# mittagessen/conformer_ocr

Measured on AMD Instinct MI355X. Metric: text lines/sec (whole node) + CER vs reference, 96×1200 bf16 batch, higher is better.
Workload: dtype bf16; 1 GPU; cfg2: conformer D=256 L=12 heads=4 sub_ch=256, batch 32 x 96x1200 per GPU, forward + CTC greedy; batches_in_queue=1, parallelism=1 independent rank(s), weights by one RCCL broadcast, streams_per_gpu=4, hipgraph_replay=True, launched_by=in-process, gpu_max_hw_queues=4, gpu_max_hw_queues_preset_by_caller=True

## Files before the change

### conformer_ocr_amd/csrc/cocr_api.hip

```cpp
#include <hip/hip_runtime.h>

#include <algorithm>
#include <cmath>
#include <cstdarg>
#include <cstdio>
#include <cstdlib>
#include <cstring>
#include <map>
#include <string>
#include <thread>
#include <vector>

#include "../../include/cocr.h"
#include "attention.hip.h"
#include "common.hip.h"
#include "conv.hip.h"
#include "ctc.hip.h"
#include "ctc_lm.hip.h"
#include "ctc_loss.hip.h"
#include "ctc_align.hip.h"
#include "train.hip.h"
#include "train_enc.hip.h"
#include "gemm.hip.h"
#include "ffn.hip.h"
#include "rowchain_args.hip.h"
#include "pack.hip.h"
#include "frontend.hip.h"
#include "norm.hip.h"
#include "preproc.hip.h"
#include "page.hip.h"
#include "augment.hip.h"
#include "score.hip.h"

static thread_local char g_err[512] = "";
static int fail(int code, const char *fmt, ...) {
    va_list ap;
    va_start(ap, fmt);
    vsnprintf(g_err, sizeof(g_err), fmt, ap);
    va_end(ap);
    return code;
}
#define HIP_TRY(expr)                                                                                      \
    do {                                                                                                   \
        hipError_t e_ = (expr);                                                                            \
        if (e_ != hipSuccess) return fail(COCR_EHIP, "%s failed: %s (%s:%d)", #expr, hipGetErrorString(e_), __FILE__, __LINE__); \
    } while (0)

extern "C" const char *cocr_last_error(void) { return g_err; }
#ifndef COCR_SRC_HASH
#define COCR_SRC_HASH "unknown"
#endif
extern "C" const char *cocr_version(void) { return "cocr-hip 0.2 (gfx950) src=" COCR_SRC_HASH; }

struct HostTensor {
    std::vector<float> data;
    std::vector<int64_t> shape;
    bool set = false;
};

struct FfnW { size_t ln_g, ln_b, w1, b1, w2, b2; };
struct LayerW {
    FfnW ffn[2];
    size_t a_ln_g, a_ln_b, wqkv, bqkv, ub, vb, wpos, wo, bo;
    size_t c_ln_g, c_ln_b, wpw1, bpw1, dww, dwb, wpw2, bpw2;
    size_t f_ln_g, f_ln_b;
};
struct StageW { size_t dw_w, dw_b, pw_w, pw_b; };
struct BlobPlan {
    size_t w0, b0;
    std::vector<StageW> stages;
    size_t wout, bout;
    std::vector<LayerW> layers;
    size_t wdec, bdec;
    size_t total = 0;
};

template <typename E> struct DevBuf {
    E *p = nullptr;
    size_t n = 0;
    const bool pinned;
    explicit DevBuf(bool pinned_ = false) : pinned(pinned_) {}
    DevBuf(const DevBuf &) = delete;
    DevBuf &operator=(const DevBuf &) = delete;
    ~DevBuf() { release(); }
    void release() {
        if (p) (void)(pinned ? hipHostFree(p) : hipFree(p));
        p = nullptr; n = 0;
    }
    hipError_t grow(size_t need, size_t alloc = 0) {
        if (need <= n) return hipSuccess;
        release();
        alloc = std::max(need, alloc);
        void *q = nullptr;
        const hipError_t e = pinned ? hipHostMalloc(&q, alloc * sizeof(E)) : hipMalloc(&q, alloc * sizeof(E));
        if (e != hipSuccess) return e;
        p = static_cast<E *>(q); n = alloc;
        return hipSuccess;
    }
};
template <typename E> static hipError_t grow_pair(DevBuf<E> &dev, DevBuf<E> &host, size_t need, size_t alloc = 0) {
    if (need <= dev.n && need <= host.n) return hipSuccess;
    dev.release(); host.release();
    hipError_t e = dev.grow(need, alloc);
    if (e == hipSuccess && (e = host.grow(need, alloc)) != hipSuccess) dev.release();
    return e;
}

#define COCR_RING_SLOTS 16
struct UploadRing {
    DevBuf<unsigned char> dev, host{true};
    hipEvent_t ev[COCR_RING_SLOTS] = {};
    int slot = 0;
    size_t at = 0;
    ~UploadRing() {
        for (hipEvent_t e : ev)
            if (e) (void)hipEventDestroy(e);
    }
    template <typename E> hipError_t stage(size_t bytes, E *&h, E *&d) {
        const size_t need = (bytes + 15) / 16 * 16 * COCR_RING_SLOTS;
        hipError_t e = hipSuccess;
        if (need > dev.n || need > host.n) {
            if ((e = hipDeviceSynchronize()) != hipSuccess) return e;
            if ((e = grow_pair(dev, host, need, (bytes + bytes / 2 + 15) / 16 * 16 * COCR_RING_SLOTS)) != hipSuccess) return e;
        }
        slot = (slot + 1) % COCR_RING_SLOTS;
        e = ev[slot] ? hipEventSynchronize(ev[slot]) : hipEventCreateWithFlags(&ev[slot], hipEventDisableTiming);
        at = dev.n / COCR_RING_SLOTS / 16 * 16 * (size_t)slot;
        h = reinterpret_cast<E *>(host.p + at); d = reinterpret_cast<E *>(dev.p + at);
        return e;
    }
    hipError_t commit(size_t bytes, hipStream_t s) {
        const hipError_t e = hipMemcpyAsync(dev.p + at, host.p + at, bytes, hipMemcpyHostToDevice, s);
        return e != hipSuccess ? e : hipEventRecord(ev[slot], s);
    }
};

struct ProfRec { int fam; hipEvent_t a, b; };
struct TrainState;

struct cocr_model {
    cocr_hparams hp;
    int device = 0;
    int D, C, L, heads, dh, dhp, ff, ksz, ncls, H, snum;
    int rD = 0, rff = 0, rdh = 0;
    bool padded = false;
    std::vector<int> feats;
    std::map<std::string, HostTensor> host;
    std::vector<std::string> names;
    int dtype = -1;
    unsigned char *blob = nullptr;
    BlobPlan plan;
    unsigned char *packed = nullptr;
    bf16_t *fpack = nullptr;
    bool packed_stale = true;
    unsigned char *ptab = nullptr;
    size_t ptab_stride = 0;
    bool ptab_stale = true;
    cocr_model *owner = nullptr;
    unsigned long long wgen = 1, seen_wgen = 0;
    std::vector<cocr_model *> sharers;
    int capN = 0, capW = 0;
    std::vector<void *> ws_allocs;
    void *z_a = nullptr, *z_b = nullptr;
    float *x = nullptr;
    void *g_lines = nullptr;
    float *g_logits = nullptr;
    void *xn = nullptr, *hid = nullptr, *q = nullptr, *k = nullptr, *vt = nullptr, *ctx = nullptr, *glu = nullptr, *dwo = nullptr;
    size_t qkv_bytes = 0;
    int vtN = -1, vtT = -1;
    int pos_maxlen = COCR_POS_MAXLEN;
    DevBuf<unsigned char> pre_buf;
    DevBuf<unsigned char> page_buf;
    UploadRing lens_ring;
    DevBuf<int32_t> ctc_lab;
    DevBuf<float> ctc_val;
    const float *amax_logits = nullptr;
    int amax_rows = 0;
    bool amax_ok = false;
    DevBuf<float> tr_pad;
    DevBuf<unsigned char> beam_bp;
    DevBuf<unsigned char> lm_scratch;
    UploadRing target_ring;
    DevBuf<float> loss_ws;
    DevBuf<unsigned> align_ws;
    UploadRing score_ring;
    DevBuf<unsigned> score_ws;
    int score_lds_max = 64 * 1024;
    int lastN = 0, lastT = 0;
    DevBuf<float> tr_part;
    float *tr_state = nullptr;
    long tr_step = 0;
    int tr_kind = -1;
    bool use_graph = false;
    struct GraphEntry { const void *lines; float *logits; int N, W, dtype; hipStream_t s; hipGraphExec_t exec; int rows; };
    std::vector<GraphEntry> graphs, graph_seen;
    bool debug = false;
    unsigned long long *stamps = nullptr;
    bool no_pad = false;
    bool beam_ref = false;
    bool no_front96 = false;
    bool no_front32 = false;
    bool no_dw_fuse = false;
    int chain_rows = 0;
    bool no_front_chain = false;
    bool ffn_probe = false;
    int att_resident_min = 192;
    bool att_resident_long = false;
    bool att_tiled = false;
    bool no_kskip = false;
    bool chain_xcd = true;
    bool no_chain = false;
    std::map<std::string, std::pair<float *, int64_t>> taps;
    DevBuf<float> tapbuf;
    TrainState *train = nullptr;
    bool profile = false;
    std::vector<ProfRec> prof;
    std::vector<hipEvent_t> ev_pool;
};

static const char *FAMILIES[] = {"frontend_fused", "frontend_conv12", "frontend_dw", "gemm_front_pw", "gemm_front_out", "layernorm",
                                 "gemm_ffn_up", "gemm_ffn_down", "ffn_fused", "chain_ffn_qkv", "chain_front_ffn_qkv", "chain_attn_out_glu", "chain_pw2_ffn_ffn_qkv", "chain_pw2_ffn", "gemm_qkv", "attention", "gemm_attn_out", "gemm_glu",
                                 "dwconv", "gemm_pw2", "gemm_decoder", "ctc_greedy", "ctc_beam", "ctc_loss", "ffn_probe", "event_pair_overhead"};
enum { FAM_FRONT96, FAM_CONV12, FAM_FDW, FAM_FPW, FAM_FOUT, FAM_LN, FAM_FFN_UP, FAM_FFN_DOWN, FAM_FFN_FUSED, FAM_CH_FIRST, FAM_CH_FRONT, FAM_CH_A, FAM_CH_B, FAM_CH_LAST, FAM_QKV, FAM_ATTN, FAM_AOUT, FAM_GLU,
       FAM_DW, FAM_PW2, FAM_DEC, FAM_GREEDY, FAM_BEAM, FAM_LOSS, FAM_FFN_PROBE, FAM_EMPTY, FAM_COUNT };

static void drop_graphs(cocr_model *m) {
    for (auto &g : m->graphs) (void)hipGraphExecDestroy(g.exec);
    m->graphs.clear();
    m->graph_seen.clear();
}

static int out_len1(int l) { return l >= 1 ? (l - 1) / 2 + 1 : 0; }

extern "C" int32_t cocr_out_len(int32_t in_len, int32_t subsampling_factor) {
    int n = 0;
    for (int f = subsampling_factor; f > 1; f >>= 1) ++n;
    for (int i = 0; i < n; ++i) in_len = out_len1(in_len);
    return in_len;
}

static void add_name(cocr_model *m, const std::string &n) { m->names.push_back(n); m->host[n]; }

struct Switch { const char *name; bool cocr_model::*flag; int cocr_model::*count; };
static const Switch SWITCHES[] = {
    {"COCR_NO_PAD", &cocr_model::no_pad, nullptr},
    {"COCR_NO_CHAIN", &cocr_model::no_chain, nullptr},
    {"COCR_NO_FRONT_CHAIN", &cocr_model::no_front_chain, nullptr},
    {"COCR_FFN_PROBE", &cocr_model::ffn_probe, nullptr},
    {"COCR_ATT_TILED", &cocr_model::att_tiled, nullptr},
    {"COCR_ATT_RESIDENT_LONG", &cocr_model::att_resident_long, nullptr},
    {"COCR_CHAIN_XCD", &cocr_model::chain_xcd, nullptr},
    {"COCR_NO_KSKIP", &cocr_model::no_kskip, nullptr},
    {"COCR_NO_DW_FUSE", &cocr_model::no_dw_fuse, nullptr},
    {"COCR_NO_FRONT96", &cocr_model::no_front96, nullptr},
    {"COCR_NO_FRONT32", &cocr_model::no_front32, nullptr},
    {"COCR_BEAM_REF", &cocr_model::beam_ref, nullptr},
    {"COCR_ATT_RESIDENT_MIN", nullptr, &cocr_model::att_resident_min},
    {"COCR_CHAIN_ROWS", nullptr, &cocr_model::chain_rows},
    {"COCR_SCORE_LDS_MAX", nullptr, &cocr_model::score_lds_max},
};

extern "C" int cocr_create(const cocr_hparams *hp, int device, cocr_model **out) {
    if (!hp || !out) return fail(COCR_EINVAL, "null argument");
    if (hp->num_classes < 1 || hp->height < 1 || hp->encoder_dim < 1 || hp->num_encoder_layers < 1 || hp->num_attention_heads < 1)
        return fail(COCR_EINVAL, "non-positive hyper-parameter");
    if (hp->encoder_dim % hp->num_attention_heads) return fail(COCR_EINVAL, "d_model %% num_heads should be zero.");
    if ((hp->conv_kernel_size - 1) % 2 || hp->conv_kernel_size < 1) return fail(COCR_EINVAL, "kernel_size should be a odd number for 'SAME' padding");
    if (hp->conv_expansion_factor != 2) return fail(COCR_EINVAL, "Currently, Only Supports expansion_factor 2");
    int sf = hp->subsampling_factor, snum = 0;
    if (sf < 2 || (sf & (sf - 1))) return fail(COCR_EINVAL, "Sampling factor should be a power of 2.");
    for (int f = sf; f > 1; f >>= 1) ++snum;
    if (snum < 1) return fail(COCR_EINVAL, "subsampling_factor must be at least 2");
    if (hp->encoder_dim % 16) return fail(COCR_EUNSUPPORTED, "encoder_dim must be a multiple of 16 (GLU tile pairing, 16-byte rows)");
    if (hp->subsampling_conv_channels % 8) return fail(COCR_EUNSUPPORTED, "subsampling_conv_channels must be a multiple of 8");
    if (hp->encoder_dim > COCR_LN_MAX_D) return fail(COCR_EUNSUPPORTED, "encoder_dim > 1024");
    const int dh = hp->encoder_dim / hp->num_attention_heads;
    if (dh > 128) return fail(COCR_EUNSUPPORTED, "d_head > 128");
    cocr_model *m = new cocr_model();
    m->hp = *hp;
    m->device = device;
    m->D = hp->encoder_dim; m->C = hp->subsampling_conv_channels; m->L = hp->num_encoder_layers;
    m->heads = hp->num_attention_heads; m->dh = dh; m->dhp = round_up(dh, 32);
    m->ff = hp->feed_forward_expansion_factor * hp->encoder_dim; m->ksz = hp->conv_kernel_size;
    m->rD = m->D; m->rff = m->ff; m->rdh = m->dh;
    m->ncls = hp->num_classes; m->H = hp->height; m->snum = snum;
    for (const Switch &w : SWITCHES) {
        const char *e = getenv(w.name);
        if (!e) continue;
        if (w.count) m->*w.count = atoi(e);
        else m->*w.flag = m->*w.flag ? e[0] != '0' : e[0] == '1';
    }
    { const char *e = getenv("COCR_CHAIN_STAMPS"); if (e && e[0] == '1') { (void)hipHostMalloc((void **)&m->stamps, 4096 * 8); memset(m->stamps, 0, 4096 * 8); } }
    int f = hp->height;
    for (int i = 0; i < snum; ++i) { f = out_len1(f); m->feats.push_back(f); }
    char buf[256];
    add_name(m, "encoder.conv_subsample.conv.0.weight");
    add_name(m, "encoder.conv_subsample.conv.0.bias");
    for (int s = 0, idx = 2; s < snum - 1; ++s, idx += 3) {
        for (int j = 0; j < 2; ++j) {
            snprintf(buf, sizeof buf, "encoder.conv_subsample.conv.%d.weight", idx + j); add_name(m, buf);
            snprintf(buf, sizeof buf, "encoder.conv_subsample.conv.%d.bias", idx + j); add_name(m, buf);
        }
    }
    add_name(m, "encoder.conv_subsample.out.0.weight");
    add_name(m, "encoder.conv_subsample.out.0.bias");
    for (int l = 0; l < m->L; ++l) {
        auto nm = [&](const char *suffix) { snprintf(buf, sizeof buf, "encoder.layers.%d.sequential.%s", l, suffix); add_name(m, buf); };
        for (int w = 0; w < 2; ++w) {
            const char *pre = w == 0 ? "0" : "3";
            for (const char *s : {"module.sequential.0.weight", "module.sequential.0.bias", "module.sequential.1.linear.weight",
                                  "module.sequential.1.linear.bias", "module.sequential.4.linear.weight", "module.sequential.4.linear.bias"}) {
                char b2[200]; snprintf(b2, sizeof b2, "%s.%s", pre, s); nm(b2);
            }
        }
        for (const char *s : {"1.module.layer_norm.weight", "1.module.layer_norm.bias", "1.module.attention.u_bias", "1.module.attention.v_bias",
                              "1.module.attention.query_proj.linear.weight", "1.module.attention.query_proj.linear.bias",
                              "1.module.attention.key_proj.linear.weight", "1.module.attention.key_proj.linear.bias",
                              "1.module.attention.value_proj.linear.weight", "1.module.attention.value_proj.linear.bias",
                              "1.module.attention.pos_proj.linear.weight", "1.module.attention.out_proj.linear.weight",
                              "1.module.attention.out_proj.linear.bias",
                              "2.module.sequential.0.weight", "2.module.sequential.0.bias", "2.module.sequential.2.conv.weight",
                              "2.module.sequential.2.conv.bias", "2.module.sequential.4.conv.weight", "2.module.sequential.5.weight",
                              "2.module.sequential.5.bias", "2.module.sequential.5.running_mean", "2.module.sequential.5.running_var",
                              "2.module.sequential.7.conv.weight", "2.module.sequential.7.conv.bias", "4.weight", "4.bias"})
            nm(s);
    }
    add_name(m, "decoder.weight");
    add_name(m, "decoder.bias");
    *out = m;
    return COCR_OK;
}

static void free_workspace(cocr_model *m) {
    for (void *p : m->ws_allocs) (void)hipFree(p);
    m->ws_allocs.clear();
    m->capN = m->capW = 0;
    m->vtN = m->vtT = -1;
}
static void clear_taps(cocr_model *m) {
    for (auto &kv : m->taps) (void)hipFree(kv.second.first);
    m->taps.clear();
    m->tapbuf.release();
}

static void drop_weights(cocr_model *m) {
    if (!m->owner) {
        for (void *p : {(void *)m->blob, (void *)m->packed, (void *)m->ptab, (void *)m->fpack})
            if (p) (void)hipFree(p);
    } else {
        auto &sh = m->owner->sharers;
        sh.erase(std::remove(sh.begin(), sh.end(), m), sh.end());
    }
    m->owner = nullptr;
    m->blob = m->packed = m->ptab = nullptr;
    m->fpack = nullptr;
}

static void train_free(cocr_model *m);
extern "C" void cocr_destroy(cocr_model *m) {
    if (!m) return;
    (void)hipSetDevice(m->device);
    train_free(m);
    free_workspace(m);
    clear_taps(m);
    for (cocr_model *sh : m->sharers) {
        drop_graphs(sh);
        sh->owner = nullptr;
        sh->blob = sh->packed = sh->ptab = nullptr;
        sh->fpack = nullptr;
    }
    m->sharers.clear();
    drop_weights(m);
    if (m->stamps) {
        (void)hipDeviceSynchronize();
        if (m->stamps[1024]) {
            for (int w = 0; w < 8; ++w) {
                const unsigned long long *q = m->stamps + 1024 + 64 * w;
                fprintf(stderr, "chain wave %d (start +%llu):", w, q[0] - m->stamps[1024]);
                for (int i = 1; i < 64 && q[i]; ++i) fprintf(stderr, " %llu", q[i] - q[i - 1]);
                fprintf(stderr, "  total %llu\n", [&] { int i = 1; while (i < 64 && q[i]) ++i; return q[i - 1] - q[0]; }());
            }
        }
        fprintf(stderr, "frontend stamps:");
        for (int i = 129; i < 192 && m->stamps[i]; ++i) fprintf(stderr, " %llu", m->stamps[i] - m->stamps[128]);
        fprintf(stderr, "\nbeam walk cycles of the stay wave, then of extension wave 0 (pairs + reads, keys, barrier + ranks, update, tail):");
        for (int i = 240; i < 250 && m->stamps[i]; ++i) fprintf(stderr, " %llu", m->stamps[i]);
        fprintf(stderr, "\nattention stamps:");
        for (int i = 193; i < 240 && m->stamps[i]; ++i) fprintf(stderr, " %llu", m->stamps[i] - m->stamps[192]);
        fprintf(stderr, "\n");
        {
            const unsigned long long *w = m->stamps + 192 + 64;
            unsigned long long t0 = ~0ull, t1 = 0;
            int nwg = 0;
            for (int i = 0; i < 1200 && w[3 * i]; ++i) { t0 = std::min(t0, w[3 * i]); t1 = std::max(t1, w[3 * i + 1]); nwg = i + 1; }
            if (nwg) {
                fprintf(stderr, "attention workgroups %d, span %.2f us (100 MHz ticks)\n", nwg, (t1 - t0) * 0.01);
                std::map<unsigned long long, int> per_cu;
                int hist_start[32] = {0};
                double dur = 0;
                for (int i = 0; i < nwg; ++i) {
                    const unsigned long long hw = w[3 * i + 2];
                    const unsigned long long cu = ((hw >> 32) << 16) | ((hw >> 8) & 0xff) | (((hw >> 13) & 7) << 8);
                    per_cu[cu]++;
                    hist_start[std::min<unsigned long long>((w[3 * i] - t0) / 100, 31)]++;
                    dur += (w[3 * i + 1] - w[3 * i]) * 0.01;
                }
                fprintf(stderr, "  mean workgroup duration %.2f us; distinct CUs %zu; start-time histogram (1 us bins):", dur / nwg, per_cu.size());
                for (int b = 0; b < 32; ++b) fprintf(stderr, " %d", hist_start[b]);
                int cnt[8] = {0};
                for (auto &kv : per_cu) cnt[std::min(kv.second, 7)]++;
                fprintf(stderr, "\n  CUs by number of workgroups received (0..7+):");
                for (int b = 0; b < 8; ++b) fprintf(stderr, " %d", cnt[b]);
                fprintf(stderr, "\n");
            }
        }
        (void)hipHostFree(m->stamps);
    }
    if (m->tr_state) (void)hipFree(m->tr_state);
    drop_graphs(m);
    for (auto &r : m->prof) { (void)hipEventDestroy(r.a); (void)hipEventDestroy(r.b); }
    for (auto e : m->ev_pool) (void)hipEventDestroy(e);
    delete m;
}

extern "C" int cocr_set_tensor(cocr_model *m, const char *name, const void *host, int dtype, int ndim, const int64_t *shape) {
    if (!m || !name || !host) return fail(COCR_EINVAL, "null argument");
    std::string n(name);
    if (n.size() > 20 && n.compare(n.size() - 19, 19, "num_batches_tracked") == 0) return COCR_OK;
    auto it = m->host.find(n);
    if (it == m->host.end()) return fail(COCR_EINVAL, "unexpected key '%s'", name);
    if (dtype != COCR_F32) return fail(COCR_EINVAL, "tensor '%s': only float32 state is accepted", name);
    int64_t cnt = 1;
    for (int i = 0; i < ndim; ++i) cnt *= shape[i];
    it->second.shape.assign(shape, shape + ndim);
    it->second.data.assign((const float *)host, (const float *)host + cnt);
    it->second.set = true;
    return COCR_OK;
}

extern "C" int cocr_missing_tensors(cocr_model *m, char *buf, size_t buflen) {
    if (!m) return fail(COCR_EINVAL, "null argument");
    int cnt = 0;
    std::string s;
    for (auto &n : m->names)
        if (!m->host[n].set) { ++cnt; s += n; s += '\n'; }
    if (buf && buflen) { strncpy(buf, s.c_str(), buflen - 1); buf[buflen - 1] = 0; }
    return cnt;
}

static size_t esize(int dtype) { return dtype == COCR_BF16 ? 2 : 4; }

static BlobPlan make_plan(const cocr_model *m, int dtype) {
    BlobPlan p;
    size_t off = 0;
    auto take = [&](size_t bytes) { size_t o = off; off += (bytes + 255) / 256 * 256; return o; };
    const size_t es = esize(dtype);
    const int D = m->D, C = m->C, ff = m->ff;
    p.w0 = take((size_t)C * 9 * 4); p.b0 = take((size_t)C * 4);
    for (int s = 0; s < m->snum - 1; ++s) {
        StageW st;
        st.dw_w = take((size_t)C * 9 * 4); st.dw_b = take((size_t)C * 4);
        st.pw_w = take((size_t)C * C * es); st.pw_b = take((size_t)C * 4);
        p.stages.push_back(st);
    }
    const int F = m->feats.back();
    p.wout = take((size_t)D * F * C * es); p.bout = take((size_t)D * 4);
    for (int l = 0; l < m->L; ++l) {
        LayerW w;
        for (int i = 0; i < 2; ++i) {
            w.ffn[i].ln_g = take(D * 4); w.ffn[i].ln_b = take(D * 4);
            w.ffn[i].w1 = take((size_t)ff * D * es); w.ffn[i].b1 = take((size_t)ff * 4);
            w.ffn[i].w2 = take((size_t)D * ff * es); w.ffn[i].b2 = take(D * 4);
        }
        w.a_ln_g = take(D * 4); w.a_ln_b = take(D * 4);
        w.wqkv = take((size_t)3 * D * D * es); w.bqkv = take((size_t)3 * D * 4);
        w.ub = take(D * 4); w.vb = take(D * 4);
        w.wpos = take((size_t)D * D * 4);
        w.wo = take((size_t)D * D * es); w.bo = take(D * 4);
        w.c_ln_g = take(D * 4); w.c_ln_b = take(D * 4);
        w.wpw1 = take((size_t)2 * D * D * es); w.bpw1 = take((size_t)2 * D * 4);
        w.dww = take((size_t)m->ksz * D * 4); w.dwb = take(D * 4);
        w.wpw2 = take((size_t)D * D * es); w.bpw2 = take(D * 4);
        w.f_ln_g = take(D * 4); w.f_ln_b = take(D * 4);
        p.layers.push_back(w);
    }
    p.wdec = take((size_t)m->ncls * D * es); p.bdec = take((size_t)m->ncls * 4);
    p.total = off;
    return p;
}

static uint16_t f32_to_bf16(float f) {
    uint32_t u;
    memcpy(&u, &f, 4);
    if ((u & 0x7fffffffu) > 0x7f800000u) return (uint16_t)((u >> 16) | 0x40);
    u += 0x7fffu + ((u >> 16) & 1u);
    return (uint16_t)(u >> 16);
}

static void put_matrix(unsigned char *dst, int dtype, const float *src, int rows, int cols, const std::vector<int> *rowmap = nullptr,
                       const std::vector<int> *colmap = nullptr) {
    for (int r = 0; r < rows; ++r) {
        const float *s = src + (size_t)(rowmap ? (*rowmap)[r] : r) * cols;
        for (int c = 0; c < cols; ++c) {
            const float v = s[colmap ? (*colmap)[c] : c];
            if (dtype == COCR_BF16) ((uint16_t *)dst)[(size_t)r * cols + c] = f32_to_bf16(v);
            else ((float *)dst)[(size_t)r * cols + c] = v;
        }
    }
}
static void put_f32(unsigned char *dst, const float *src, size_t n) { memcpy(dst, src, n * 4); }

static int expect_shape(const cocr_model *m, const std::string &name, std::initializer_list<int64_t> shape, const HostTensor **out) {
    auto it = m->host.find(name);
    if (it == m->host.end() || !it->second.set) return fail(COCR_ESTATE, "missing tensor '%s'", name.c_str());
    if (it->second.shape != std::vector<int64_t>(shape)) {
        std::string got;
        for (auto v : it->second.shape) got += std::to_string(v) + ",";
        return fail(COCR_EINVAL, "size mismatch for %s: got (%s)", name.c_str(), got.c_str());
    }
    *out = &it->second;
    return COCR_OK;
}

static int ensure_ptab(cocr_model *m, hipStream_t s);

static void free_workspace(cocr_model *m);
static int set_engine_dims(cocr_model *m, int dtype) {
    const int wide = m->rD < 256 ? 256 : 512;
    const int slot = m->heads > 0 && wide % m->heads == 0 ? wide / m->heads : 0;
    const bool pad = dtype == COCR_BF16 && !m->no_pad && m->rD >= 128 && m->rD < 512 && m->rD != 256 && slot >= m->rdh && slot % 32 == 0 && slot <= 128 &&
                     round_up(m->rff, 256) <= (wide == 256 ? 1024 : 2048);
    const int D = pad ? wide : m->rD, ff = pad ? round_up(m->rff, 256) : m->rff, dh = pad ? slot : m->rdh, dhp = pad ? slot : round_up(m->rdh, 32);
    if (D != m->D || ff != m->ff || dh != m->dh || dhp != m->dhp) {
        HIP_TRY(hipDeviceSynchronize());
        drop_graphs(m);
        free_workspace(m);
        m->capN = m->capW = 0;
    }
    m->D = D; m->ff = ff; m->dh = dh; m->dhp = dhp; m->padded = pad;
    return COCR_OK;
}

static int alloc_blob(cocr_model *m, int dtype) {
    if (dtype != COCR_BF16 && dtype != COCR_F32) return fail(COCR_EINVAL, "compute dtype must be COCR_BF16 or COCR_F32");
    HIP_TRY(hipSetDevice(m->device));
    { const int rc = set_engine_dims(m, dtype); if (rc) return rc; }
    drop_weights(m);
    m->wgen++;
    m->ptab_stale = true;
    if (m->tr_state) { (void)hipFree(m->tr_state); m->tr_state = nullptr; m->tr_step = 0; }
    m->packed_stale = true;
    m->plan = make_plan(m, dtype);
    m->dtype = dtype;
    HIP_TRY(hipMalloc((void **)&m->blob, m->plan.total));
    HIP_TRY(hipMemset(m->blob, 0, m->plan.total));
    return COCR_OK;
}

extern "C" int cocr_finalize_empty(cocr_model *m, int compute_dtype) {
    if (!m) return fail(COCR_EINVAL, "null argument");
    int rc = alloc_blob(m, compute_dtype);
    if (rc) return rc;
    HIP_TRY(hipDeviceSynchronize());
    return COCR_OK;
}

extern "C" int cocr_share_weights(cocr_model *m, cocr_model *owner) {
    if (!m || !owner || m == owner) return fail(COCR_EINVAL, "two different models expected");
    if (owner->owner) return fail(COCR_EINVAL, "the owner itself shares another model's weights");
    if (owner->dtype < 0 || !owner->blob) return fail(COCR_ESTATE, "the owner is not finalized");
    if (m->device != owner->device || memcmp(&m->hp, &owner->hp, sizeof m->hp) != 0) return fail(COCR_EINVAL, "models of the same hyper-parameters on the same device expected");
    if (m->train || owner->train) return fail(COCR_ESTATE, "not while a training state exists");
    HIP_TRY(hipSetDevice(m->device));
    HIP_TRY(hipDeviceSynchronize());
    if (m->dtype != owner->dtype || !m->blob || m->owner) { const int rc = alloc_blob(m, owner->dtype); if (rc) return rc; }
    drop_weights(m);
    m->owner = owner;
    owner->sharers.push_back(m);
    m->seen_wgen = 0;
    m->blob = owner->blob;
    drop_graphs(m);
    return COCR_OK;
}

extern "C" int cocr_weight_blob(cocr_model *m, void **device_ptr, size_t *bytes) {
    if (!m || !device_ptr || !bytes) return fail(COCR_EINVAL, "null argument");
    if (!m->blob) return fail(COCR_ESTATE, "model not finalized");
    if (m->owner) return fail(COCR_ESTATE, "this model shares another model's weights: address the owner");
    *device_ptr = m->blob;
    *bytes = m->plan.total;
    m->packed_stale = m->ptab_stale = true;
    return COCR_OK;
}

extern "C" int cocr_blob_export(cocr_model *m, void *dst_device, size_t bytes, void *stream) {
    if (!m || !dst_device) return fail(COCR_EINVAL, "null argument");
    if (!m->blob) return fail(COCR_ESTATE, "model not finalized");
    if (m->owner) return fail(COCR_ESTATE, "this model shares another model's weights: address the owner");
    if (bytes != m->plan.total) return fail(COCR_EINVAL, "blob is %zu bytes, buffer %zu", m->plan.total, bytes);
    HIP_TRY(hipSetDevice(m->device));
    HIP_TRY(hipMemcpyAsync(dst_device, m->blob, bytes, hipMemcpyDeviceToDevice, (hipStream_t)stream));
    return COCR_OK;
}
extern "C" int cocr_blob_import(cocr_model *m, const void *src_device, size_t bytes, void *stream) {
    if (!m || !src_device) return fail(COCR_EINVAL, "null argument");
    if (!m->blob) return fail(COCR_ESTATE, "model not finalized");
    if (bytes != m->plan.total) return fail(COCR_EINVAL, "blob is %zu bytes, buffer %zu", m->plan.total, bytes);
    if (m->owner) return fail(COCR_ESTATE, "this model shares another model's weights: address the owner");
    HIP_TRY(hipSetDevice(m->device));
    HIP_TRY(hipMemcpyAsync(m->blob, src_device, bytes, hipMemcpyDeviceToDevice, (hipStream_t)stream));
    m->packed_stale = m->ptab_stale = true;
    if (m->tr_state) { (void)hipFree(m->tr_state); m->tr_state = nullptr; m->tr_step = 0; }
    return COCR_OK;
}

static void put_mapped(unsigned char *dst, int dtype, const float *src, int src_cols, const std::vector<int> &rmap, const std::vector<int> &cmap) {
    const size_t vcols = cmap.size();
    for (size_t r = 0; r < rmap.size(); ++r)
        for (size_t c = 0; c < vcols; ++c) {
            const float v = (rmap[r] >= 0 && cmap[c] >= 0) ? src[(size_t)rmap[r] * src_cols + cmap[c]] : 0.0f;
            if (dtype == COCR_BF16) ((uint16_t *)dst)[r * vcols + c] = f32_to_bf16(v);
            else ((float *)dst)[r * vcols + c] = v;
        }
}
static void put_vec(unsigned char *dst, const float *src, const std::vector<int> &map) {
    for (size_t i = 0; i < map.size(); ++i) ((float *)dst)[i] = map[i] >= 0 ? src[map[i]] : 0.0f;
}

extern "C" int cocr_finalize(cocr_model *m, int dtype) {
    if (!m) return fail(COCR_EINVAL, "null argument");
    if (dtype != COCR_BF16 && dtype != COCR_F32) return fail(COCR_EINVAL, "compute dtype must be COCR_BF16 or COCR_F32");
    HIP_TRY(hipSetDevice(m->device));
    int rc;
    if ((rc = set_engine_dims(m, dtype))) return rc;
    const int rD = m->rD, rff = m->rff, rdh = m->rdh, D = m->D, C = m->C, ff = m->ff, k = m->ksz, h = m->heads, dh = m->dh;
    std::vector<int> Mm(D), Fm(ff), Am(D), Gm((size_t)2 * D), ident_cls(m->ncls);
    for (int c = 0; c < D; ++c) Mm[c] = c < rD ? c : -1;
    for (int c = 0; c < ff; ++c) Fm[c] = c < rff ? c : -1;
    for (int c = 0; c < D; ++c) Am[c] = (c / dh < h && c % dh < rdh) ? (c / dh) * rdh + c % dh : -1;
    for (int n = 0; n < 2 * D; ++n) {
        const int tn = n >> 4, c = n & 15, j = tn >> 1, v = 16 * j + c;
        Gm[n] = v < rD ? ((tn & 1) ? rD + v : v) : -1;
    }
    for (int c = 0; c < m->ncls; ++c) ident_cls[c] = c;
    const BlobPlan plan = make_plan(m, dtype);
    std::vector<unsigned char> stage(plan.total, 0);
    unsigned char *st = stage.data();
    const HostTensor *t = nullptr;
    char buf[256];
#define GET(NAME, ...)                                          \
    if ((rc = expect_shape(m, NAME, {__VA_ARGS__}, &t))) return rc;
    GET("encoder.conv_subsample.conv.0.weight", C, 1, 3, 3); put_f32(st + plan.w0, t->data.data(), (size_t)C * 9);
    GET("encoder.conv_subsample.conv.0.bias", C); put_f32(st + plan.b0, t->data.data(), C);
    for (int s = 0, idx = 2; s < m->snum - 1; ++s, idx += 3) {
        snprintf(buf, sizeof buf, "encoder.conv_subsample.conv.%d.weight", idx); GET(buf, C, 1, 3, 3); put_f32(st + plan.stages[s].dw_w, t->data.data(), (size_t)C * 9);
        snprintf(buf, sizeof buf, "encoder.conv_subsample.conv.%d.bias", idx); GET(buf, C); put_f32(st + plan.stages[s].dw_b, t->data.data(), C);
        snprintf(buf, sizeof buf, "encoder.conv_subsample.conv.%d.weight", idx + 1); GET(buf, C, C, 1, 1); put_matrix(st + plan.stages[s].pw_w, dtype, t->data.data(), C, C);
        snprintf(buf, sizeof buf, "encoder.conv_subsample.conv.%d.bias", idx + 1); GET(buf, C); put_f32(st + plan.stages[s].pw_b, t->data.data(), C);
    }
    {
        const int F = m->feats.back();
        GET("encoder.conv_subsample.out.0.weight", rD, (int64_t)C * F);
        std::vector<int> colmap((size_t)F * C);
        for (int f = 0; f < F; ++f) for (int c = 0; c < C; ++c) colmap[(size_t)f * C + c] = c * F + f;
        put_mapped(st + plan.wout, dtype, t->data.data(), F * C, Mm, colmap);
        GET("encoder.conv_subsample.out.0.bias", rD); put_vec(st + plan.bout, t->data.data(), Mm);
    }
    for (int l = 0; l < m->L; ++l) {
        const LayerW &w = plan.layers[l];
        auto key = [&](const char *suffix) { snprintf(buf, sizeof buf, "encoder.layers.%d.sequential.%s", l, suffix); return std::string(buf); };
        for (int i = 0; i < 2; ++i) {
            const std::string pre = std::string(i == 0 ? "0" : "3") + ".module.sequential.";
            GET(key((pre + "0.weight").c_str()), rD); put_vec(st + w.ffn[i].ln_g, t->data.data(), Mm);
            GET(key((pre + "0.bias").c_str()), rD); put_vec(st + w.ffn[i].ln_b, t->data.data(), Mm);
            GET(key((pre + "1.linear.weight").c_str()), rff, rD); put_mapped(st + w.ffn[i].w1, dtype, t->data.data(), rD, Fm, Mm);
            GET(key((pre + "1.linear.bias").c_str()), rff); put_vec(st + w.ffn[i].b1, t->data.data(), Fm);
            GET(key((pre + "4.linear.weight").c_str()), rD, rff); put_mapped(st + w.ffn[i].w2, dtype, t->data.data(), rff, Mm, Fm);
            GET(key((pre + "4.linear.bias").c_str()), rD); put_vec(st + w.ffn[i].b2, t->data.data(), Mm);
        }
        GET(key("1.module.layer_norm.weight"), rD); put_vec(st + w.a_ln_g, t->data.data(), Mm);
        GET(key("1.module.layer_norm.bias"), rD); put_vec(st + w.a_ln_b, t->data.data(), Mm);
        const char *proj[3] = {"query", "key", "value"};
        for (int j = 0; j < 3; ++j) {
            snprintf(buf, sizeof buf, "encoder.layers.%d.sequential.1.module.attention.%s_proj.linear.weight", l, proj[j]);
            GET(std::string(buf), rD, rD); put_mapped(st + w.wqkv + (size_t)j * D * D * esize(dtype), dtype, t->data.data(), rD, Am, Mm);
            snprintf(buf, sizeof buf, "encoder.layers.%d.sequential.1.module.attention.%s_proj.linear.bias", l, proj[j]);
            GET(std::string(buf), rD); put_vec(st + w.bqkv + (size_t)j * D * 4, t->data.data(), Am);
        }
        GET(key("1.module.attention.u_bias"), h, rdh); put_vec(st + w.ub, t->data.data(), Am);
        GET(key("1.module.attention.v_bias"), h, rdh); put_vec(st + w.vb, t->data.data(), Am);
        GET(key("1.module.attention.pos_proj.linear.weight"), rD, rD); put_mapped(st + w.wpos, COCR_F32, t->data.data(), rD, Am, Mm);
        GET(key("1.module.attention.out_proj.linear.weight"), rD, rD); put_mapped(st + w.wo, dtype, t->data.data(), rD, Mm, Am);
        GET(key("1.module.attention.out_proj.linear.bias"), rD); put_vec(st + w.bo, t->data.data(), Mm);
        GET(key("2.module.sequential.0.weight"), rD); put_vec(st + w.c_ln_g, t->data.data(), Mm);
        GET(key("2.module.sequential.0.bias"), rD); put_vec(st + w.c_ln_b, t->data.data(), Mm);
        GET(key("2.module.sequential.2.conv.weight"), 2 * rD, rD, 1); put_mapped(st + w.wpw1, dtype, t->data.data(), rD, Gm, Mm);
        GET(key("2.module.sequential.2.conv.bias"), 2 * rD); put_vec(st + w.bpw1, t->data.data(), Gm);
        {
            const HostTensor *wd, *g, *b, *mu, *var;
            if ((rc = expect_shape(m, key("2.module.sequential.4.conv.weight"), {rD, 1, k}, &wd))) return rc;
            if ((rc = expect_shape(m, key("2.module.sequential.5.weight"), {rD}, &g))) return rc;
            if ((rc = expect_shape(m, key("2.module.sequential.5.bias"), {rD}, &b))) return rc;
            if ((rc = expect_shape(m, key("2.module.sequential.5.running_mean"), {rD}, &mu))) return rc;
            if ((rc = expect_shape(m, key("2.module.sequential.5.running_var"), {rD}, &var))) return rc;
            float *tw = (float *)(st + w.dww), *tb = (float *)(st + w.dwb);
            for (int c = 0; c < rD; ++c) {
                const float s = g->data[c] / sqrtf(var->data[c] + 1e-5f);
                for (int tau = 0; tau < k; ++tau) tw[(size_t)tau * D + c] = wd->data[(size_t)c * k + tau] * s;
                tb[c] = b->data[c] - mu->data[c] * s;
            }
        }
        GET(key("2.module.sequential.7.conv.weight"), rD, rD, 1); put_mapped(st + w.wpw2, dtype, t->data.data(), rD, Mm, Mm);
        GET(key("2.module.sequential.7.conv.bias"), rD); put_vec(st + w.bpw2, t->data.data(), Mm);
        GET(key("4.weight"), rD); put_vec(st + w.f_ln_g, t->data.data(), Mm);
        GET(key("4.bias"), rD); put_vec(st + w.f_ln_b, t->data.data(), Mm);
    }
    GET("decoder.weight", m->ncls, rD); put_mapped(st + plan.wdec, dtype, t->data.data(), rD, ident_cls, Mm);
    GET("decoder.bias", m->ncls); put_f32(st + plan.bdec, t->data.data(), m->ncls);
#undef GET
    if ((rc = alloc_blob(m, dtype))) return rc;
    HIP_TRY(hipMemcpy(m->blob, st, plan.total, hipMemcpyHostToDevice));
    if ((rc = ensure_ptab(m, nullptr))) return rc;
    HIP_TRY(hipDeviceSynchronize());
    return COCR_OK;
}

template <typename T> static int compute_pos_tables(cocr_model *m, hipStream_t s) {
    const int D = m->D, rD = m->rD, maxlen = m->pos_maxlen, R = 2 * maxlen - 1;
    std::vector<float> pe((size_t)R * D, 0.0f);
    for (int r = 0; r < R; ++r) {
        const float pos = (float)(maxlen - 1 - r);
        for (int i = 0; i < rD; i += 2) {
            const float div = expf((float)i * (float)(-(log(10000.0) / rD)));
            const float ang = pos * div;
            pe[(size_t)r * D + i] = sinf(ang);
            if (i + 1 < rD) pe[(size_t)r * D + i + 1] = cosf(ang);
        }
    }
    float *d_pe = nullptr;
    HIP_TRY(hipMalloc((void **)&d_pe, pe.size() * 4));
    HIP_TRY(hipMemcpyAsync(d_pe, pe.data(), pe.size() * 4, hipMemcpyHostToDevice, s));
    for (int l = 0; l < m->L; ++l) {
        EpiPosTable<T> epi{(T *)(m->ptab + (size_t)l * m->ptab_stride), m->dh, m->dhp, m->heads};
        HIP_TRY(launch_gemm<float>(s, d_pe, D, (const float *)(m->blob + m->plan.layers[l].wpos), D, R, D, D, epi));
    }
    HIP_TRY(hipStreamSynchronize(s));
    HIP_TRY(hipFree(d_pe));
    return COCR_OK;
}
static int ensure_ptab(cocr_model *m, hipStream_t s) {
    if (!m->ptab_stale) return COCR_OK;
    m->ptab_stride = (size_t)(2 * m->pos_maxlen - 1) * m->heads * m->dhp * esize(m->dtype);
    if (!m->ptab) {
        HIP_TRY(hipMalloc((void **)&m->ptab, m->ptab_stride * m->L));
        HIP_TRY(hipMemsetAsync(m->ptab, 0, m->ptab_stride * m->L, s));
    }
    int rc = m->dtype == COCR_BF16 ? compute_pos_tables<bf16_t>(m, s) : compute_pos_tables<float>(m, s);
    if (rc) return rc;
    m->ptab_stale = false;
    return COCR_OK;
}

static int ws_alloc(cocr_model *m, void **p, size_t bytes) {
    HIP_TRY(hipMalloc(p, bytes ? bytes : 256));
    m->ws_allocs.push_back(*p);
    return COCR_OK;
}

extern "C" int cocr_reserve(cocr_model *m, int N, int W) {
    if (!m) return fail(COCR_EINVAL, "null argument");
    if (m->dtype < 0) return fail(COCR_ESTATE, "model not finalized");
    if (N < 1 || W < 1) return fail(COCR_EINVAL, "empty batch");
    if (N <= m->capN && W <= m->capW) return COCR_OK;
    HIP_TRY(hipSetDevice(m->device));
    HIP_TRY(hipDeviceSynchronize());
    N = std::max(N, m->capN); W = std::max(W, m->capW);
    drop_graphs(m);
    free_workspace(m);
    const size_t es = esize(m->dtype);
    int T = W;
    for (int i = 0; i < m->snum; ++i) T = out_len1(T);
    const int Tz = m->snum >= 2 ? out_len1(out_len1(W)) : out_len1(W);
    const size_t M = (size_t)N * T, Tp = round_up(T, 64);
    int rc;
    const size_t zbytes = (size_t)N * Tz * m->feats[m->snum >= 2 ? 1 : 0] * m->C * es;
    if ((rc = ws_alloc(m, &m->z_a, zbytes))) return rc;
    if ((rc = ws_alloc(m, &m->z_b, zbytes))) return rc;
    if ((rc = ws_alloc(m, (void **)&m->x, (M + 128) * m->D * 4))) return rc;
    if ((rc = ws_alloc(m, &m->xn, M * m->D * es))) return rc;
    if ((rc = ws_alloc(m, &m->hid, M * m->ff * es))) return rc;
    m->qkv_bytes = (size_t)N * m->heads * Tp * m->dhp * es;
    if ((rc = ws_alloc(m, &m->q, m->qkv_bytes))) return rc;
    if ((rc = ws_alloc(m, &m->k, m->qkv_bytes))) return rc;
    if ((rc = ws_alloc(m, &m->vt, m->qkv_bytes))) return rc;
    if ((rc = ws_alloc(m, &m->ctx, M * m->D * es))) return rc;
    if ((rc = ws_alloc(m, &m->glu, M * m->D * es))) return rc;
    if ((rc = ws_alloc(m, &m->dwo, M * m->D * es))) return rc;
    if ((rc = ws_alloc(m, &m->g_lines, (size_t)N * m->H * W * 4))) return rc;
    if ((rc = ws_alloc(m, (void **)&m->g_logits, M * m->ncls * 4))) return rc;
    m->capN = N; m->capW = W;
    return COCR_OK;
}

template <typename T> __global__ void to_f32_kernel(const T *in, float *out, size_t n) {
    for (size_t i = (size_t)blockIdx.x * blockDim.x + threadIdx.x; i < n; i += (size_t)gridDim.x * blockDim.x) out[i] = to_f32(in[i]);
}
template <typename T> __global__ void tap_narrow_kernel(const T *in, float *out, size_t rows, int D, int rD, int dh, int rdh, int head_major) {
    for (size_t i = (size_t)blockIdx.x * blockDim.x + threadIdx.x; i < rows * rD; i += (size_t)gridDim.x * blockDim.x) {
        const size_t r = i / rD;
        const int c = (int)(i - r * rD);
        out[i] = to_f32(in[r * D + (head_major ? (c / rdh) * dh + c % rdh : c)]);
    }
}
template <typename T> static int tap(cocr_model *m, hipStream_t s, const std::string &name, const T *src, size_t n) {
    if (!m->debug) return COCR_OK;
    auto ends = [&](const char *suf) { const size_t l = strlen(suf); return name.size() >= l && name.compare(name.size() - l, l, suf) == 0; };
    const bool own_layout = ends(".q") || ends(".k") || ends(".v") || ends(".z2") || ends(".z3");
    const bool narrow = m->padded && !own_layout && n % (size_t)m->D == 0;
    const size_t nout = narrow ? n / m->D * m->rD : n;
    float *dst = nullptr;
    HIP_TRY(hipMalloc((void **)&dst, nout * 4));
    if (narrow) hipLaunchKernelGGL((tap_narrow_kernel<T>), dim3(256), dim3(256), 0, s, src, dst, n / m->D, m->D, m->rD, m->dh, m->rdh, ends(".ctx") ? 1 : 0);
    else hipLaunchKernelGGL((to_f32_kernel<T>), dim3(256), dim3(256), 0, s, src, dst, n);
    HIP_TRY(hipStreamSynchronize(s));
    auto it = m->taps.find(name);
    if (it != m->taps.end()) (void)hipFree(it->second.first);
    m->taps[name] = {dst, (int64_t)nout};
    return COCR_OK;
}

extern "C" int cocr_set_debug(cocr_model *m, int on) {
    if (!m) return fail(COCR_EINVAL, "null argument");
    m->debug = on != 0;
    if (!on) clear_taps(m);
    return COCR_OK;
}
extern "C" int cocr_debug_tap(cocr_model *m, const char *name, float *host_out, int64_t max_elems, int64_t *n_elems) {
    if (!m || !name) return fail(COCR_EINVAL, "null argument");
    auto it = m->taps.find(name);
    if (it == m->taps.end()) return fail(COCR_EINVAL, "no tap '%s' (debug off, or stage not run)", name);
    if (n_elems) *n_elems = it->second.second;
    if (host_out) {
        if (max_elems < it->second.second) return fail(COCR_EINVAL, "tap '%s' has %lld elements", name, (long long)it->second.second);
        HIP_TRY(hipMemcpy(host_out, it->second.first, it->second.second * 4, hipMemcpyDeviceToHost));
    }
    return COCR_OK;
}

struct ProfScope {
    cocr_model *m; hipStream_t s; ProfRec r; bool on;
    ProfScope(cocr_model *m_, hipStream_t s_, int fam) : m(m_), s(s_), on(m_->profile) {
        if (!on) return;
        r.fam = fam;
        auto get = [&]() { hipEvent_t e; if (m->ev_pool.empty()) { (void)hipEventCreate(&e); } else { e = m->ev_pool.back(); m->ev_pool.pop_back(); } return e; };
        r.a = get(); r.b = get();
        (void)hipEventRecord(r.a, s);
    }
    ~ProfScope() { if (on) { (void)hipEventRecord(r.b, s); m->prof.push_back(r); } }
};

extern "C" int cocr_profile(cocr_model *m, int on) {
    if (!m) return fail(COCR_EINVAL, "null argument");
    m->profile = on != 0;
    for (auto &r : m->prof) { m->ev_pool.push_back(r.a); m->ev_pool.push_back(r.b); }
    m->prof.clear();
    return COCR_OK;
}
extern "C" int cocr_profile_read(cocr_model *m, char *names, size_t names_len, double *ms, int64_t *launches, int max_entries) {
    if (!m) return fail(COCR_EINVAL, "null argument");
    HIP_TRY(hipSetDevice(m->device));
    HIP_TRY(hipDeviceSynchronize());
    double sum[FAM_COUNT] = {0};
    int64_t cnt[FAM_COUNT] = {0};
    for (auto &r : m->prof) {
        float t = 0.f;
        HIP_TRY(hipEventElapsedTime(&t, r.a, r.b));
        sum[r.fam] += t; cnt[r.fam]++;
    }
    std::string s;
    int n = 0;
    for (int f = 0; f < FAM_COUNT && n < max_entries; ++f) {
        if (!cnt[f]) continue;
        s += FAMILIES[f]; s += '\n';
        ms[n] = sum[f] / (double)cnt[f]; launches[n] = cnt[f];
        ++n;
    }
    if (names && names_len) { strncpy(names, s.c_str(), names_len - 1); names[names_len - 1] = 0; }
    return n;
}

#define LAUNCH_CHECK() HIP_TRY(hipGetLastError())

#define GEMM_TRY(call)                                                                                 \
    do {                                                                                               \
        hipError_t e_ = (call);                                                                        \
        if (e_ != hipSuccess) return fail(COCR_EHIP, "kernel launch failed: %s (%s:%d)", hipGetErrorString(e_), __FILE__, __LINE__); \
    } while (0)

template <typename T, int DHP>
static hipError_t launch_attention(hipStream_t s, int N, const T *q, const T *k, const T *v, const T *ptab, const float *ub,
                                   const float *vb, T *ctx, int Tn, int Tp, int heads, int dh, float scale, int pos_center, unsigned long long *stamps = nullptr,
                                   bool tiled_only = false, int resident_min = 192, bool resident_long = false) {
    if constexpr (sizeof(T) == 2 && DHP == 64) {
        const int ntiles = ceil_div(Tn, 16), nqb = ceil_div(ntiles, AF_QT);
        if (dh == DHP && (Tn <= AF_TK || resident_long) && !tiled_only && !stamps && nqb * N * heads >= resident_min) {
            const int Tk0 = round_up(Tn, 64), npass = ceil_div(Tk0, AF_TK), Tk = round_up(ceil_div(Tk0, npass), 64);
            const int ntw = ceil_div(ntiles, nqb);
            const size_t lds = (size_t)(2 * Tk + 16 * ntw + Tk) * 128 + AF_WAVES * AF_SROWS * AF_SK * sizeof(float);
            auto kern = npass > 1 ? relpos_attention_full_kernel<true> : relpos_attention_full_kernel<false>;
            hipError_t e = raise_lds_limit((const void *)kern, lds);
            if (e != hipSuccess) return e;
            hipLaunchKernelGGL(kern, dim3(nqb, N * heads), dim3(64 * AF_WAVES), lds, s, (const bf16_t *)q, (const bf16_t *)k, (const bf16_t *)v,
                               (const bf16_t *)ptab, ub, vb, (bf16_t *)ctx, Tn, Tp, heads, scale * 1.44269504088896340736f, pos_center, ntw, Tk);
            return hipGetLastError();
        }
    }
    const size_t lds = attention_lds_bytes<T, DHP>();
    auto kern = relpos_attention_kernel<T, DHP>;
    hipError_t e = raise_lds_limit((const void *)kern, lds);
    if (e != hipSuccess) return e;
    hipLaunchKernelGGL(kern, dim3(ceil_div(Tn, 64), N * heads), dim3(256), lds, s, q, k, v, ptab, ub, vb, ctx, Tn, Tp, heads, dh,
                       scale * 1.44269504088896340736f, pos_center, stamps);
    return hipGetLastError();
}

static int ensure_ctc_scratch(cocr_model *m, size_t rows);

enum FrontForm {
    FRONT_96,
    FRONT_CONV0,
    FRONT_PW32,
    FRONT_MFMA,
    FRONT_VALU,
};
enum OutForm {
    OUT_IN_CHAIN,
    OUT_SPLITK,
    OUT_GEMM,
};
struct Form {
    FrontForm front;
    OutForm out;
    bool rowln;
    bool chain;
    bool ffn_fused;
    bool dw_fused;
    bool taps;
    bool argmax;
    int chain_rows;
};

static int hw_queue_count() {
    static const int n = [] {
        const char *e = getenv("GPU_MAX_HW_QUEUES");
        char *end = nullptr;
        long v = e ? strtol(e, &end, 10) : 4;
        if (e && (end == e || *end)) v = 4;
        return (int)std::min(32L, std::max(1L, v));
    }();
    return n;
}

static int chain_rows_for(const cocr_model *m, int M) {
    const bool d256 = m->D == 256;
    auto form = [&](int hint) { return 16 * (d256 ? rowchain_pick_mt<256>(M, hint) : rowchain_pick_mt<512>(M, hint)); };
    if (m->chain_rows > 0) return form(m->chain_rows);
    const cocr_model *root = m->owner ? m->owner : m;
    const int S = 1 + (int)root->sharers.size();
    if (S < 2) return form(0);
    const int Q = std::max(1, hw_queue_count() - 1), turns = ceil_div(S, Q);
    static const int forms256[] = {96, 64, 48}, forms512[] = {64};
    const int *forms = d256 ? forms256 : forms512, nforms = d256 ? 3 : 1;
    int rows = 32;
    for (int i = 0; i < nforms; ++i) {
        if (M < 50 * forms[i]) continue;
        rows = forms[i];
        if ((long)ceil_div(M, rows) * S >= 256L * turns) break;
    }
    return rows;
}

#ifndef COCR_FO_SPLITS
#define COCR_FO_SPLITS 2
#endif
static Form forward_form(const cocr_model *m, int N, int W) {
    const bool bf16 = m->dtype == COCR_BF16, f2only = m->snum == 1;
    const int es = bf16 ? 2 : 4, D = m->D, C = m->C, H = m->H;
    const int T1 = out_len1(W), T2 = f2only ? T1 : out_len1(T1), F2 = m->feats[f2only ? 0 : 1];
    const int Kf = m->feats.back() * C, M = N * cocr_out_len(W, m->hp.subsampling_factor);
    const size_t lds32 = (size_t)(4 * 16 + 3) * ((H + 11) & ~3) * 4 + (size_t)16 * F2 * 80;
    Form f{};
    f.taps = m->debug;
    f.rowln = bf16 ? gemm_rowln_supported<bf16_t>(D) : gemm_rowln_supported<float>(D);
    f.chain = bf16 && rowchain_supported(D, m->ff, m->dh) && !m->no_chain;
    if (bf16 && m->snum == 2 && frontend96_supported(C, m->feats[0], m->feats[1], H) && !m->no_front96) f.front = FRONT_96;
    else if (f2only) f.front = FRONT_CONV0;
    else if (bf16 && C == 32 && F2 <= 32 && lds32 <= 160 * 1024 && !f.taps && !m->no_front32) f.front = FRONT_PW32;
    else f.front = bf16 && C % 64 == 0 ? FRONT_MFMA : FRONT_VALU;
    if (f.chain && Kf % 256 == 0 && !m->no_front_chain) f.out = OUT_IN_CHAIN;
    else if (f.rowln && Kf % (COCR_FO_SPLITS * (128 / es)) == 0 && D <= 256 && (size_t)COCR_FO_SPLITS * M * D * 4 <= (size_t)N * T2 * F2 * C * es)
        f.out = OUT_SPLITK;
    else f.out = OUT_GEMM;
    f.ffn_fused = bf16 && f.rowln && ffn_fused_supported<int>(D, m->ff);
    f.dw_fused = m->ksz == 31 && (!m->no_dw_fuse || f.taps);
    f.argmax = m->ncls <= 128 && D % (128 / es) == 0;
    f.chain_rows = f.chain ? chain_rows_for(m, M) : 0;
    return f;
}

template <typename T> struct Fwd {
    cocr_model *m;
    const Form &f;
    hipStream_t s;
    const BlobPlan &P;
    const int N, W, D, T1, T2, F1, F2, Tn, M, Tp;
    const float ffr, scale;
    T *const za, *const zb;
    float *const x;
    T *const xn, *const hid, *const q, *const k, *const v, *const ctx, *const glu, *const dwo;
    Fwd(cocr_model *m_, const Form &f_, int N_, int W_, hipStream_t s_)
        : m(m_), f(f_), s(s_), P(m_->plan), N(N_), W(W_), D(m_->D), T1(out_len1(W_)), T2(m_->snum == 1 ? T1 : out_len1(T1)), F1(m_->feats[0]),
          F2(m_->feats[m_->snum == 1 ? 0 : 1]), Tn(cocr_out_len(W_, m_->hp.subsampling_factor)), M(N_ * Tn), Tp(round_up(Tn, 64)),
          ffr(m_->hp.half_step_residual ? 0.5f : 1.0f), scale(1.0f / sqrtf((float)m_->rdh)), za((T *)m_->z_a), zb((T *)m_->z_b), x(m_->x),
          xn((T *)m_->xn), hid((T *)m_->hid), q((T *)m_->q), k((T *)m_->k), v((T *)m_->vt), ctx((T *)m_->ctx), glu((T *)m_->glu), dwo((T *)m_->dwo) {}
    const float *F32(size_t off) const { return (const float *)(m->blob + off); }
    const T *WT(size_t off) const { return (const T *)(m->blob + off); }
    template <typename S> int tap(int l, const char *what, const S *src, size_t n) const {
        if (!f.taps) return COCR_OK;
        char nm[64];
        if (l < 0) snprintf(nm, sizeof nm, "%s", what);
        else snprintf(nm, sizeof nm, "l%d.%s", l, what);
        return ::tap<S>(m, s, nm, src, n);
    }
    int tap_x(int l, const char *what, const float *src) const { return tap<float>(l, what, src, (size_t)M * D); }
    int tap_qkv(int l) const {
        const size_t n = m->qkv_bytes / sizeof(T);
        int rc;
        if ((rc = tap<T>(l, "q", q, n)) || (rc = tap<T>(l, "k", k, n)) || (rc = tap<T>(l, "v", v, n))) return rc;
        return COCR_OK;
    }
};

template <typename T, typename TIn> static int frontend(const Fwd<T> &c, const TIn *lines) {
    cocr_model *m = c.m;
    const BlobPlan &P = c.P;
    const hipStream_t s = c.s;
    const int N = c.N, H = m->H, W = c.W, C = m->C, T1 = c.T1, F1 = c.F1, T2 = c.T2, F2 = c.F2;
    const FrontForm form = c.f.front;
    T *za = c.za, *zb = c.zb;
    int rc;
    if (form == FRONT_CONV0) {
        ProfScope ps(m, s, FAM_CONV12);
        const size_t npos = (size_t)N * T1 * F1;
        hipLaunchKernelGGL((frontend_conv0_kernel<T, TIn>), dim3((unsigned)((npos * (size_t)(C / 2) + 255) / 256)), dim3(256), 0, s, lines, H, W, T1, F1, C, npos,
                           c.F32(P.w0), c.F32(P.b0), zb);
        LAUNCH_CHECK();
        return COCR_OK;
    }
    if (form == FRONT_96) {
        ProfScope ps(m, s, FAM_FRONT96);
        const size_t n0 = (size_t)(C / 16) * 64 * 4;
        GEMM_TRY(launch_frontend96<TIn>(s, lines, N, H, W, T1, F1, T2, m->fpack, c.F32(P.b0), m->fpack + n0, c.F32(P.stages[0].dw_b),
                                        (const bf16_t *)(m->packed + P.stages[0].pw_w), c.F32(P.stages[0].pw_b), (bf16_t *)zb, m->stamps ? m->stamps + 128 : nullptr));
    } else if (form == FRONT_PW32) {
        ProfScope ps(m, s, FAM_CONV12);
        const size_t lds = (size_t)(4 * 16 + 3) * ((H + 11) & ~3) * 4 + (size_t)16 * F2 * 80;
        auto kern = frontend_conv12pw32_kernel<TIn>;
        GEMM_TRY(raise_lds_limit((const void *)kern, lds));
        hipLaunchKernelGGL(kern, dim3(ceil_div(T2, 16), N), dim3(256), lds, s, lines, H, W, T1, F1, T2, F2, c.F32(P.w0), c.F32(P.b0),
                           c.F32(P.stages[0].dw_w), c.F32(P.stages[0].dw_b), (const bf16_t *)c.WT(P.stages[0].pw_w), c.F32(P.stages[0].pw_b), (bf16_t *)zb);
        LAUNCH_CHECK();
    } else {
        {
            ProfScope ps(m, s, FAM_CONV12);
            if (form == FRONT_MFMA) {
                GEMM_TRY(launch_conv12_mfma<TIn>(s, lines, N, H, W, T1, F1, T2, F2, C, c.F32(P.w0), c.F32(P.b0), c.F32(P.stages[0].dw_w), c.F32(P.stages[0].dw_b),
                                                 (bf16_t *)za));
            } else {
                const int TB = std::max(1, 512 / C);
                const size_t lds = (size_t)(4 * TB + 3) * ((H + 11) & ~3) * 4;
                hipLaunchKernelGGL((frontend_conv12_kernel<T, TIn>), dim3(ceil_div(T2, TB), N), dim3(256), lds, s, lines, H, W, T1, F1, T2, F2, C,
                                   c.F32(P.w0), c.F32(P.b0), c.F32(P.stages[0].dw_w), c.F32(P.stages[0].dw_b), za, TB);
                LAUNCH_CHECK();
            }
        }
        if ((rc = c.tap(-1, "front.z2", za, (size_t)N * T2 * F2 * C))) return rc;
        ProfScope ps(m, s, FAM_FPW);
        EpiBiasAct<T, ACT_RELU> epi{zb, C, c.F32(P.stages[0].pw_b), C};
        GEMM_TRY(launch_gemm<T>(s, za, C, c.WT(P.stages[0].pw_w), C, N * T2 * F2, C, C, epi));
    }
    if ((rc = c.tap(-1, "front.z3", zb, (size_t)N * T2 * F2 * C))) return rc;
    int Tc = T2, Fc = F2;
    for (int st = 1; st < m->snum - 1; ++st) {
        const int To = out_len1(Tc), Fo = m->feats[st + 1];
        {
            ProfScope ps(m, s, FAM_FDW);
            hipLaunchKernelGGL((dw3x3s2_kernel<T>), dim3(1024), dim3(256), 0, s, zb, N, Tc, Fc, To, Fo, C, c.F32(P.stages[st].dw_w),
                               c.F32(P.stages[st].dw_b), za);
            LAUNCH_CHECK();
        }
        {
            ProfScope ps(m, s, FAM_FPW);
            EpiBiasAct<T, ACT_RELU> epi{zb, C, c.F32(P.stages[st].pw_b), C};
            GEMM_TRY(launch_gemm<T>(s, za, C, c.WT(P.stages[st].pw_w), C, N * To * Fo, C, C, epi));
        }
        Tc = To; Fc = Fo;
    }
    return COCR_OK;
}

template <typename T> static int layernorm(const Fwd<T> &c, size_t g1, size_t b1, bool write_f32, long g2, long b2) {
    ProfScope ps(c.m, c.s, FAM_LN);
    launch_layernorm<T>(c.s, c.x, c.M, c.D, c.F32(g1), c.F32(b1), write_f32 ? c.x : nullptr, g2 >= 0 ? c.F32((size_t)g2) : nullptr,
                        b2 >= 0 ? c.F32((size_t)b2) : nullptr, c.xn, c.m->rD);
    LAUNCH_CHECK();
    return COCR_OK;
}

template <typename T> static int gemm_to_stream(const Fwd<T> &c, int fam, const T *A, int K, size_t w, size_t bias, float alpha, bool resid,
                                                size_t g1, size_t b1, long g2, long b2) {
    const int M = c.M, D = c.D;
    {
        ProfScope ps(c.m, c.s, fam);
        if (c.f.rowln) {
            EpiResidualLN<T, 1> e{c.x, D, c.F32(bias), alpha, D, resid ? 1 : 0, c.F32(g1), c.F32(b1), g2 >= 0 ? c.F32((size_t)g2) : nullptr,
                                  b2 >= 0 ? c.F32((size_t)b2) : nullptr, c.xn};
            e.Dn = c.m->rD;
            GEMM_TRY(launch_gemm_rowln<T>(c.s, A, K, c.WT(w), K, M, D, K, e));
            return COCR_OK;
        }
        if (resid) { EpiResidual e{c.x, D, c.F32(bias), alpha, D}; GEMM_TRY(launch_gemm<T>(c.s, A, K, c.WT(w), K, M, D, K, e)); }
        else { EpiStoreF32 e{c.x, D, c.F32(bias), D}; GEMM_TRY(launch_gemm<T>(c.s, A, K, c.WT(w), K, M, D, K, e)); }
    }
    return layernorm(c, g1, b1, g2 >= 0, g2, b2);
}

template <typename T> static int front_out(const Fwd<T> &c) {
    cocr_model *m = c.m;
    const BlobPlan &P = c.P;
    const FfnW &f0 = P.layers[0].ffn[0];
    const int Kf = m->feats.back() * m->C, M = c.M, D = c.D;
    if (c.f.out == OUT_IN_CHAIN) return COCR_OK;
    if (c.f.out == OUT_SPLITK) {
        float *partial = reinterpret_cast<float *>(c.za);
        { ProfScope ps(m, c.s, FAM_FOUT); GEMM_TRY(launch_gemm_splitk<T>(c.s, c.zb, Kf, c.WT(P.wout), Kf, M, D, Kf, COCR_FO_SPLITS, partial)); }
        ProfScope ps(m, c.s, FAM_LN);
        hipLaunchKernelGGL((splitk_reduce_ln_kernel<T>), dim3(ceil_div(M, 16)), dim3(256), 0, c.s, partial, COCR_FO_SPLITS, (size_t)M * D, c.F32(P.bout), M, D,
                           m->rD, c.F32(f0.ln_g), c.F32(f0.ln_b), c.x, c.xn);
        LAUNCH_CHECK();
    } else {
        const int rc = gemm_to_stream(c, FAM_FOUT, c.zb, Kf, P.wout, P.bout, 1.0f, false, f0.ln_g, f0.ln_b, -1, -1);
        if (rc) return rc;
    }
    return c.tap_x(-1, "front.y", c.x);
}

template <typename T> static int ffn_up(const Fwd<T> &c, const FfnW &fw) {
    ProfScope ps(c.m, c.s, FAM_FFN_UP);
    EpiBiasAct<T, ACT_SILU> e{c.hid, c.m->ff, c.F32(fw.b1), c.m->ff};
    GEMM_TRY(launch_gemm<T>(c.s, c.xn, c.D, c.WT(fw.w1), c.D, c.M, c.m->ff, c.D, e));
    return COCR_OK;
}
template <typename T> static int ffn(const Fwd<T> &c, const FfnW &fw, size_t g1, size_t b1, long g2, long b2) {
    if constexpr (sizeof(T) == 2) {
        if (c.f.ffn_fused) {
            ProfScope ps(c.m, c.s, FAM_FFN_FUSED);
            EpiResidualLN<T, 1> e{c.x, c.D, c.F32(fw.b2), c.ffr, c.D, 1, c.F32(g1), c.F32(b1), g2 >= 0 ? c.F32((size_t)g2) : nullptr,
                                  b2 >= 0 ? c.F32((size_t)b2) : nullptr, c.xn};
            GEMM_TRY(launch_ffn_fused(c.s, (const bf16_t *)c.xn, (const bf16_t *)c.WT(fw.w1), c.F32(fw.b1), (const bf16_t *)c.WT(fw.w2), c.M, c.D, c.m->ff, e));
            return COCR_OK;
        }
    }
    const int rc = ffn_up(c, fw);
    return rc ? rc : gemm_to_stream(c, FAM_FFN_DOWN, c.hid, c.m->ff, fw.w2, fw.b2, c.ffr, true, g1, b1, g2, b2);
}

template <typename T, int DHP> static hipError_t attention_dhp(const Fwd<T> &c, int l, unsigned long long *stamps) {
    const cocr_model *m = c.m;
    const LayerW &w = c.P.layers[l];
    return launch_attention<T, DHP>(c.s, c.N, c.q, c.k, c.v, (const T *)(m->ptab + (size_t)l * m->ptab_stride), c.F32(w.ub), c.F32(w.vb), c.ctx, c.Tn,
                                    c.Tp, m->heads, m->dh, c.scale, m->pos_maxlen - 1, stamps, m->att_tiled, m->att_resident_min, m->att_resident_long);
}
template <typename T> static int attention(const Fwd<T> &c, int l, unsigned long long *stamps) {
    ProfScope ps(c.m, c.s, FAM_ATTN);
    const int dhp = c.m->dhp;
    GEMM_TRY((dhp == 32   ? attention_dhp<T, 32>(c, l, stamps)
              : dhp == 64 ? attention_dhp<T, 64>(c, l, stamps)
              : dhp == 96 ? attention_dhp<T, 96>(c, l, stamps)
                          : attention_dhp<T, 128>(c, l, stamps)));
    return COCR_OK;
}

template <typename T> static int dwconv(const Fwd<T> &c, const LayerW &w) {
    ProfScope ps(c.m, c.s, FAM_DW);
    launch_dwconv<T>(c.s, c.glu, c.N, c.Tn, c.D, c.m->ksz, c.F32(w.dww), c.F32(w.dwb), c.dwo);
    LAUNCH_CHECK();
    return COCR_OK;
}

template <typename T> static int encoder_products(const Fwd<T> &c) {
    cocr_model *m = c.m;
    const hipStream_t s = c.s;
    const int M = c.M, D = c.D;
    const size_t MD = (size_t)M * D;
    int rc;
    for (int l = 0; l < m->L; ++l) {
        const LayerW &w = c.P.layers[l];
        const bool last = l + 1 == m->L;
        const long g_next = last ? -1 : (long)c.P.layers[l + 1].ffn[0].ln_g, b_next = last ? -1 : (long)c.P.layers[l + 1].ffn[0].ln_b;
        if ((rc = ffn(c, w.ffn[0], w.a_ln_g, w.a_ln_b, -1, -1)) || (rc = c.tap_x(l, "ffn1", c.x))) return rc;
        { ProfScope ps(m, s, FAM_QKV); EpiQKV<T> e{c.q, c.k, c.v, c.F32(w.bqkv), D, m->dh, m->dhp, m->heads, c.Tn, c.Tp, 3 * D}; GEMM_TRY(launch_gemm<T>(s, c.xn, D, c.WT(w.wqkv), D, M, 3 * D, D, e)); }
        if ((rc = attention(c, l, nullptr)) || (rc = c.tap_qkv(l)) || (rc = c.tap(l, "ctx", c.ctx, MD))) return rc;
        if ((rc = gemm_to_stream(c, FAM_AOUT, c.ctx, D, w.wo, w.bo, 1.0f, true, w.c_ln_g, w.c_ln_b, -1, -1)) || (rc = c.tap_x(l, "mhsa", c.x))) return rc;
        { ProfScope ps(m, s, FAM_GLU); EpiGLU<T> e{c.glu, D, c.F32(w.bpw1), 2 * D}; GEMM_TRY(launch_gemm<T>(s, c.xn, D, c.WT(w.wpw1), D, M, 2 * D, D, e)); }
        if ((rc = dwconv(c, w)) || (rc = c.tap(l, "glu", c.glu, MD)) || (rc = c.tap(l, "dw", c.dwo, MD))) return rc;
        if ((rc = gemm_to_stream(c, FAM_PW2, c.dwo, D, w.wpw2, w.bpw2, 1.0f, true, w.ffn[1].ln_g, w.ffn[1].ln_b, -1, -1)) || (rc = c.tap_x(l, "conv", c.x))) return rc;
        if (!c.f.taps) {
            if ((rc = ffn(c, w.ffn[1], w.f_ln_g, w.f_ln_b, g_next, b_next))) return rc;
            continue;
        }
        if ((rc = ffn_up(c, w.ffn[1]))) return rc;
        { ProfScope ps(m, s, FAM_FFN_DOWN); EpiResidual e{c.x, D, c.F32(w.ffn[1].b2), c.ffr, D}; GEMM_TRY(launch_gemm<T>(s, c.hid, m->ff, c.WT(w.ffn[1].w2), m->ff, M, D, m->ff, e)); }
        if ((rc = c.tap_x(l, "ffn2", c.x)) || (rc = layernorm(c, w.f_ln_g, w.f_ln_b, true, g_next, b_next)) || (rc = c.tap_x(l, "out", c.x))) return rc;
    }
    return COCR_OK;
}

template <typename T> static int encoder_chains(const Fwd<T> &c) {
    cocr_model *m = c.m;
    const BlobPlan &P = c.P;
    const int D = c.D, M = c.M;
    const size_t MD = (size_t)M * D;
    const bool taps = c.f.taps;
    int rc;
    float *tp[4] = {nullptr, nullptr, nullptr, nullptr};
    bf16_t *tap_dw = nullptr;
    if (taps) {
        HIP_TRY(m->tapbuf.grow(MD * 4 + MD / 2));
        for (int i = 0; i < 4; ++i) tp[i] = m->tapbuf.p + (size_t)i * MD;
        tap_dw = reinterpret_cast<bf16_t *>(m->tapbuf.p + 4 * MD);
    }
    auto CW = [&](size_t off) { return (const bf16_t *)(m->packed + off); };
    auto launch = [&](const ChainArgs &a, int fam) -> int {
        ProfScope ps(m, c.s, fam);
        GEMM_TRY(D == 256 ? launch_rowchain_256(c.s, a, taps, c.f.chain_rows) : launch_rowchain_512(c.s, a, taps, c.f.chain_rows));
        return COCR_OK;
    };
    auto base = [&](const T *A0, int nstages) {
        ChainArgs a{}; a.x = c.x; a.x_in_blocked = 1; a.x_out_blocked = 1; a.xn = (bf16_t *)c.xn; a.M = M; a.dh = m->dh; a.dhp = m->dhp; a.heads = m->heads; a.T_ = c.Tn; a.Tp = c.Tp; a.inv_d = 1.0f / (float)m->rD; a.xcd_order = m->chain_xcd ? 1 : 0;
        a.kd = (m->padded && !m->no_kskip) ? ceil_div(m->rD, 32) : 8; a.kl = (m->padded && !m->no_kskip) ? ((m->rff - 1) % 256) / 32 + 1 : 8;
        a.A0 = (const bf16_t *)A0; a.nstages = nstages; return a; };
    auto st_rowln = [&](size_t wgt, size_t bias, float alpha, size_t g1, size_t b1) {
        ChainStage st{}; st.kind = ST_ROWLN; st.W = CW(wgt); st.bias = c.F32(bias); st.N = D; st.alpha = alpha;
        st.g1 = c.F32(g1); st.b1 = c.F32(b1); return st; };
    auto st_ffn = [&](const FfnW &fw, size_t g1, size_t b1, long g2, long b2) {
        ChainStage st{}; st.kind = ST_FFN; st.W = CW(fw.w1); st.W2 = CW(fw.w2); st.bias = c.F32(fw.b1); st.bias2 = c.F32(fw.b2);
        st.N = m->ff; st.alpha = c.ffr; st.g1 = c.F32(g1); st.b1 = c.F32(b1);
        st.g2 = g2 >= 0 ? c.F32((size_t)g2) : nullptr; st.b2 = b2 >= 0 ? c.F32((size_t)b2) : nullptr; return st; };
    auto st_qkv = [&](const LayerW &lw) {
        ChainStage st{}; st.kind = ST_QKV; st.W = CW(lw.wqkv); st.bias = c.F32(lw.bqkv); st.N = 3 * D;
        st.q = (bf16_t *)c.q; st.k = (bf16_t *)c.k; st.v = (bf16_t *)c.v; return st; };
    const LayerW &w0 = P.layers[0];
    if (c.f.out == OUT_IN_CHAIN) {
        ChainArgs a = base(c.zb, 3); a.x_in_blocked = 0;
        ChainStage f{}; f.kind = ST_FRONT; f.W = CW(P.wout); f.bias = c.F32(P.bout); f.N = D; f.K = m->feats.back() * m->C; f.alpha = 1.0f;
        f.g1 = c.F32(w0.ffn[0].ln_g); f.b1 = c.F32(w0.ffn[0].ln_b);
        a.st[0] = f;
        a.st[1] = st_ffn(w0.ffn[0], w0.a_ln_g, w0.a_ln_b, -1, -1); a.st[1].store_x = 1;
        a.st[2] = st_qkv(w0);
        a.st[0].tap_pre = tp[1]; a.st[1].tap_pre = tp[0];
        if ((rc = launch(a, FAM_CH_FRONT)) || (rc = c.tap_x(-1, "front.y", tp[1])) || (rc = c.tap_x(0, "ffn1", tp[0])) || (rc = c.tap_qkv(0))) return rc;
    } else {
        ChainArgs a = base(c.xn, 2); a.x_in_blocked = 0;
        a.st[0] = st_ffn(w0.ffn[0], w0.a_ln_g, w0.a_ln_b, -1, -1); a.st[0].store_x = 1;
        a.st[1] = st_qkv(w0);
        a.st[0].tap_pre = tp[0];
        if ((rc = launch(a, FAM_CH_FIRST)) || (rc = c.tap_x(0, "ffn1", tp[0])) || (rc = c.tap_qkv(0))) return rc;
    }
    if (m->ffn_probe) {
        ChainArgs a = base(c.zb, 1);
        a.st[0] = st_ffn(w0.ffn[0], w0.a_ln_g, w0.a_ln_b, -1, -1);
        if ((rc = launch(a, FAM_FFN_PROBE))) return rc;
    }
    for (int l = 0; l < m->L; ++l) {
        const LayerW &w = P.layers[l];
        const bool last = l + 1 == m->L;
        if ((rc = attention(c, l, (m->stamps && l == 5) ? m->stamps + 192 : nullptr))) return rc;
        {
            ChainArgs a = base(c.ctx, 2);
            a.st[0] = st_rowln(w.wo, w.bo, 1.0f, w.c_ln_g, w.c_ln_b); a.st[0].store_x = 1;
            ChainStage g{}; g.kind = ST_GLU; g.W = CW(w.wpw1); g.bias = c.F32(w.bpw1); g.N = 2 * D; g.out = (bf16_t *)c.glu;
            a.st[1] = g;
            a.st[0].tap_pre = tp[0];
            if ((rc = c.tap(l, "ctx", c.ctx, MD)) || (rc = launch(a, FAM_CH_A)) || (rc = c.tap_x(l, "mhsa", tp[0])) || (rc = c.tap(l, "glu", c.glu, MD))) return rc;
        }
        if (!c.f.dw_fused && (rc = dwconv(c, w))) return rc;
        ChainArgs a = base(c.dwo, 2);
        if (c.f.dw_fused) { a.dw_in = (const bf16_t *)c.glu; a.dw_w = c.F32(w.dww); a.dw_b = c.F32(w.dwb); a.tap_dw = tap_dw; }
        a.st[0] = st_rowln(w.wpw2, w.bpw2, 1.0f, w.ffn[1].ln_g, w.ffn[1].ln_b);
        a.st[0].tap_pre = tp[0];
        if (!last) {
            const LayerW &nx = P.layers[l + 1];
            a.st[1] = st_ffn(w.ffn[1], w.f_ln_g, w.f_ln_b, (long)nx.ffn[0].ln_g, (long)nx.ffn[0].ln_b);
            a.st[2] = st_ffn(nx.ffn[0], nx.a_ln_g, nx.a_ln_b, -1, -1); a.st[2].store_x = 1;
            a.st[3] = st_qkv(nx);
            a.nstages = 4;
            a.st[1].tap_pre = tp[1]; a.st[1].tap_post = tp[2]; a.st[2].tap_pre = tp[3];
            a.stamps = (m->stamps && l == 5) ? m->stamps + 1024 : nullptr;
            if ((rc = launch(a, FAM_CH_B))) return rc;
        } else {
            a.st[1] = st_ffn(w.ffn[1], w.f_ln_g, w.f_ln_b, -1, -1); a.st[1].store_x = 1; a.st[1].store_xn = 1;
            a.st[1].tap_pre = tp[1];
            if ((rc = launch(a, FAM_CH_LAST))) return rc;
        }
        if ((rc = c.tap(l, "dw", c.f.dw_fused ? (const T *)tap_dw : (const T *)c.dwo, MD)) || (rc = c.tap_x(l, "conv", tp[0])) || (rc = c.tap_x(l, "ffn2", tp[1])))
            return rc;
        if (!last && ((rc = c.tap_x(l, "out", tp[2])) || (rc = c.tap_x(l + 1, "ffn1", tp[3])) || (rc = c.tap_qkv(l + 1)))) return rc;
        if (last && (rc = c.tap(l, "out", c.xn, MD))) return rc;
    }
    return COCR_OK;
}

template <typename T> static int decoder(const Fwd<T> &c, float *logits) {
    cocr_model *m = c.m;
    const int M = c.M, D = c.D;
    ProfScope ps(m, c.s, FAM_DEC);
    if (c.f.argmax) {
        const int rc = ensure_ctc_scratch(m, (size_t)M);
        if (rc) return rc;
        EpiLogitsArgmax e{logits, m->ncls, c.F32(c.P.bdec), m->ncls, m->ctc_lab.p, m->ctc_val.p};
        GemmArgs<T> a{c.xn, D, c.WT(c.P.wdec), D, M, m->ncls, D, 0};
        GEMM_TRY((launch_ring_cfg<T, 64, 128, 3, EpiLogitsArgmax>(c.s, a, e)));
        m->amax_ok = true; m->amax_rows = M;
        return COCR_OK;
    }
    EpiStoreF32 e{logits, m->ncls, c.F32(c.P.bdec), m->ncls};
    GEMM_TRY(launch_gemm<T>(c.s, c.xn, D, c.WT(c.P.wdec), D, M, m->ncls, D, e));
    m->amax_ok = false;
    return COCR_OK;
}

template <typename T, typename TIn>
static int forward_impl(cocr_model *m, const Form &f, const TIn *lines, int N, int W, float *logits, hipStream_t s) {
    const Fwd<T> c(m, f, N, W, s);
    { ProfScope ps(m, s, FAM_EMPTY); }
    int rc;
    if ((rc = frontend<T, TIn>(c, lines)) || (rc = front_out(c))) return rc;
    if (m->vtN != N || m->vtT != c.Tn) {
        for (T *p : {c.q, c.k, c.v}) HIP_TRY(hipMemsetAsync(p, 0, m->qkv_bytes, s));
        m->vtN = N; m->vtT = c.Tn;
    }
    if constexpr (sizeof(T) == 2) rc = f.chain ? encoder_chains(c) : encoder_products(c);
    else rc = encoder_products(c);
    return rc ? rc : decoder(c, logits);
}

static int ensure_packed(cocr_model *m, const Form &f, hipStream_t s) {
    if ((!f.chain && f.front != FRONT_96) || !m->packed_stale) return COCR_OK;
    if (!m->packed) HIP_TRY(hipMalloc((void **)&m->packed, m->plan.total));
    const int D = m->D, ff = m->ff, C = m->C;
    auto pack = [&](size_t off, int N, int K, float scale = 1.0f) {
        hipLaunchKernelGGL(pack_frag_kernel, dim3(std::min(1024, ceil_div(N * K / 8, 256))), dim3(256), 0, s, (const bf16_t *)(m->blob + off),
                           (bf16_t *)(m->packed + off), N, K, scale);
    };
    const float ffr = m->hp.half_step_residual ? 0.5f : 1.0f;
    if (f.chain)
        for (const LayerW &w : m->plan.layers) {
            for (int i = 0; i < 2; ++i) { pack(w.ffn[i].w1, ff, D); pack(w.ffn[i].w2, D, ff, ffr); }
            pack(w.wqkv, 3 * D, D); pack(w.wo, D, D); pack(w.wpw1, 2 * D, D); pack(w.wpw2, D, D);
        }
    if (f.out == OUT_IN_CHAIN) pack(m->plan.wout, D, m->feats.back() * C);
    if (f.front == FRONT_96) {
        pack(m->plan.stages[0].pw_w, C, C);
        const size_t n0 = (size_t)(C / 16) * 64 * 4, n2 = (size_t)(C / 16) * 5 * 64 * 8;
        if (!m->fpack) HIP_TRY(hipMalloc((void **)&m->fpack, (n0 + n2) * sizeof(bf16_t)));
        hipLaunchKernelGGL(frontend_pack_kernel, dim3(ceil_div((int)n2, 256)), dim3(256), 0, s, (const float *)(m->blob + m->plan.w0),
                           (const float *)(m->blob + m->plan.stages[0].dw_w), m->fpack, m->fpack + n0, C);
    }
    LAUNCH_CHECK();
    m->packed_stale = false;
    drop_graphs(m);
    return COCR_OK;
}

static int forward_entry(cocr_model *m, const void *lines, int line_dtype, int N, int H, int W, const int32_t *in_lens,
                         float *logits, int32_t *out_lens, void *stream);
extern "C" int cocr_forward(cocr_model *m, const void *lines, int line_dtype, int N, int H, int W, const int32_t *in_lens,
                            float *logits, int32_t *out_lens, void *stream) {
    if (m) m->amax_logits = nullptr;
    const int rc = forward_entry(m, lines, line_dtype, N, H, W, in_lens, logits, out_lens, stream);
    if (rc == COCR_OK && m->amax_ok) m->amax_logits = logits;
    return rc;
}
extern "C" int cocr_forget_argmax(cocr_model *m) {
    if (!m) return fail(COCR_EINVAL, "null argument");
    m->amax_logits = nullptr;
    return COCR_OK;
}
static int forward_entry(cocr_model *m, const void *lines, int line_dtype, int N, int H, int W, const int32_t *in_lens,
                         float *logits, int32_t *out_lens, void *stream) {
    if (!m || !lines || !logits) return fail(COCR_EINVAL, "null argument");
    if (m->dtype < 0 || !m->blob) return fail(COCR_ESTATE, "model not finalized");
    if (H != m->H) return fail(COCR_EINVAL, "line height %d does not match the model's height %d", H, m->H);
    if (N < 1 || W < 1) return fail(COCR_EINVAL, "empty batch");
    HIP_TRY(hipSetDevice(m->device));
    {
        const int Tp64 = round_up(cocr_out_len(W, m->hp.subsampling_factor), 64);
        if (Tp64 > 65536) return fail(COCR_EUNSUPPORTED, "more than 65536 output frames");
        cocr_model *root = m->owner ? m->owner : m;
        if (Tp64 + 64 > root->pos_maxlen) {
            HIP_TRY(hipDeviceSynchronize());
            drop_graphs(m);
            if (root->ptab) { (void)hipFree(root->ptab); root->ptab = nullptr; }
            root->pos_maxlen = round_up(Tp64 + 64, 1024);
            root->ptab_stale = true;
            root->wgen++;
        }
    }
    int rc;
    if (m->owner && (m->owner->dtype != m->dtype || m->owner->plan.total != m->plan.total)) {
        cocr_model *o = m->owner;
        if (o->dtype < 0 || !o->blob) return fail(COCR_ESTATE, "the model whose weights this one shares is not finalized");
        HIP_TRY(hipDeviceSynchronize());
        if ((rc = set_engine_dims(m, o->dtype))) return rc;
        drop_graphs(m);
        free_workspace(m);
        m->plan = make_plan(m, o->dtype);
        m->dtype = o->dtype;
        m->blob = o->blob;
        m->amax_logits = nullptr;
        m->seen_wgen = 0;
    }
    rc = cocr_reserve(m, N, W);
    if (rc) return rc;
    if (in_lens && out_lens)
        for (int i = 0; i < N; ++i) out_lens[i] = cocr_out_len(in_lens[i], m->hp.subsampling_factor);
    hipStream_t s = (hipStream_t)stream;
    const Form form = forward_form(m, N, W);
    if (m->owner) {
        cocr_model *o = m->owner;
        if (o->packed_stale || o->ptab_stale) {
            HIP_TRY(hipDeviceSynchronize());
            if ((rc = ensure_packed(o, form, s)) || (rc = ensure_ptab(o, s))) return rc;
            HIP_TRY(hipDeviceSynchronize());
            o->wgen++;
        }
        if (m->seen_wgen != o->wgen) {
            m->blob = o->blob; m->packed = o->packed; m->fpack = o->fpack; m->ptab = o->ptab; m->ptab_stride = o->ptab_stride; m->pos_maxlen = o->pos_maxlen;
            m->packed_stale = m->ptab_stale = false;
            m->seen_wgen = o->wgen;
            drop_graphs(m);
        }
    } else {
        const bool rebuilt = m->packed_stale || m->ptab_stale;
        if (rebuilt && m->wgen > 1) HIP_TRY(hipDeviceSynchronize());
        if ((rc = ensure_packed(m, form, s)) || (rc = ensure_ptab(m, s))) return rc;
        if (rebuilt) { m->wgen++; HIP_TRY(hipStreamSynchronize(s)); }
        if (m->seen_wgen != m->wgen) {
            if (m->seen_wgen) drop_graphs(m);
            m->seen_wgen = m->wgen;
        }
    }
    m->lastN = N;
    m->lastT = cocr_out_len(W, m->hp.subsampling_factor);
    auto run_on = [&](const void *in, float *out) -> int {
        if (m->dtype == COCR_BF16) {
            if (line_dtype == COCR_F32) return forward_impl<bf16_t, float>(m, form, (const float *)in, N, W, out, s);
            if (line_dtype == COCR_U8) return forward_impl<bf16_t, uint8_t>(m, form, (const uint8_t *)in, N, W, out, s);
        } else {
            if (line_dtype == COCR_F32) return forward_impl<float, float>(m, form, (const float *)in, N, W, out, s);
            if (line_dtype == COCR_U8) return forward_impl<float, uint8_t>(m, form, (const uint8_t *)in, N, W, out, s);
        }
        return fail(COCR_EINVAL, "line dtype must be COCR_F32 or COCR_U8");
    };
    auto run = [&]() -> int { return run_on(lines, logits); };
    if (line_dtype != COCR_F32 && line_dtype != COCR_U8) return fail(COCR_EINVAL, "line dtype must be COCR_F32 or COCR_U8");
    if (!m->use_graph || m->debug || m->profile || s == nullptr) return run();
    const int Tn = cocr_out_len(W, m->hp.subsampling_factor);
    const bool shape_ready = m->vtN == N && m->vtT == Tn;
    auto same = [&](const cocr_model::GraphEntry &g) { return g.lines == lines && g.logits == logits && g.N == N && g.W == W && g.dtype == line_dtype; };
    auto same_shape = [&](const cocr_model::GraphEntry &g) { return g.lines == nullptr && g.N == N && g.W == W && g.dtype == line_dtype; };
    auto capture = [&](const void *in, float *out, hipGraphExec_t *exec) -> int {
        hipGraph_t graph = nullptr;
        HIP_TRY(hipStreamBeginCapture(s, hipStreamCaptureModeThreadLocal));
        int r = run_on(in, out);
        hipError_t ce = hipStreamEndCapture(s, &graph);
        if (r) { if (graph) (void)hipGraphDestroy(graph); return r; }
        if (ce != hipSuccess) return fail(COCR_EHIP, "hipStreamEndCapture failed: %s", hipGetErrorString(ce));
        HIP_TRY(hipGraphInstantiate(exec, graph, nullptr, nullptr, 0));
        (void)hipGraphDestroy(graph);
        if (m->graphs.size() >= 16) { (void)hipGraphExecDestroy(m->graphs.front().exec); m->graphs.erase(m->graphs.begin()); }
        return COCR_OK;
    };
    const size_t in_bytes = (size_t)N * H * W * (line_dtype == COCR_F32 ? 4 : 1), out_bytes = (size_t)N * Tn * m->ncls * 4;
    auto staged_launch = [&](hipGraphExec_t exec) -> int {
        HIP_TRY(hipMemcpyAsync(m->g_lines, lines, in_bytes, hipMemcpyDefault, s));
        HIP_TRY(hipGraphLaunch(exec, s));
        HIP_TRY(hipMemcpyAsync(logits, m->g_logits, out_bytes, hipMemcpyDeviceToDevice, s));
        return COCR_OK;
    };
    for (auto &g : m->graphs)
        if (g.N == N && g.W == W && g.rows != form.chain_rows) {
            drop_graphs(m);
            break;
        }
    for (auto &g : m->graphs)
        if (same(g)) { HIP_TRY(hipGraphLaunch(g.exec, s)); return COCR_OK; }
    bool seen = false, seen_shape = false;
    for (auto &g : m->graph_seen) { seen = seen || same(g); seen_shape = seen_shape || same_shape(g); }
    if (seen && shape_ready) {
        hipGraphExec_t exec = nullptr;
        if ((rc = capture(lines, logits, &exec))) return rc;
        m->graphs.push_back({lines, logits, N, W, line_dtype, s, exec, form.chain_rows});
        HIP_TRY(hipGraphLaunch(exec, s));
        return COCR_OK;
    }
    if (m->graph_seen.size() >= 32) m->graph_seen.erase(m->graph_seen.begin());
    m->graph_seen.push_back({lines, logits, N, W, line_dtype, s, nullptr, 0});
    for (auto &g : m->graphs)
        if (same_shape(g)) return staged_launch(g.exec);
    if (!seen_shape || !shape_ready) {
        m->graph_seen.push_back({nullptr, nullptr, N, W, line_dtype, s, nullptr, 0});
        return run();
    }
    hipGraphExec_t exec = nullptr;
    if ((rc = capture(m->g_lines, m->g_logits, &exec))) return rc;
    m->graphs.push_back({nullptr, nullptr, N, W, line_dtype, s, exec, form.chain_rows});
    return staged_launch(exec);
}

extern "C" int cocr_collate_lines(const void *const *lines, const int32_t *widths, int N, int H, int elem_size, void *dst, int W, int threads) {
    if (N < 0 || H <= 0 || W <= 0 || (elem_size != 1 && elem_size != 4)) return fail(COCR_EINVAL, "collate: bad shape or element size");
    if (N == 0) return COCR_OK;
    if (!lines || !widths || !dst) return fail(COCR_EINVAL, "collate: null argument");
    for (int i = 0; i < N; ++i)
        if (!lines[i] || widths[i] < 0 || widths[i] > W) return fail(COCR_EINVAL, "collate: line %d is %d wide, the batch %d", i, widths[i], W);
    const long rows = (long)N * H;
    auto span = [=](long r0, long r1) {
        for (long r = r0; r < r1; ++r) {
            const int i = (int)(r / H), y = (int)(r % H);
            const size_t wb = (size_t)widths[i] * elem_size, Wb = (size_t)W * elem_size;
            char *d = (char *)dst + (size_t)r * Wb;
            memcpy(d, (const char *)lines[i] + (size_t)y * wb, wb);
            memset(d + wb, 0, Wb - wb);
        }
    };
    const int nt = (int)std::max(1L, std::min<long>(std::min(threads, 64), rows / 64));
    if (nt <= 1) { span(0, rows); return COCR_OK; }
    std::vector<std::thread> pool;
    pool.reserve(nt - 1);
    for (int t = 1; t < nt; ++t) pool.emplace_back(span, rows * t / nt, rows * (t + 1) / nt);
    span(0, rows / nt);
    for (auto &t : pool) t.join();
    return COCR_OK;
}

static int upload_lens(cocr_model *m, const int32_t *lens, int N, hipStream_t s, const int32_t *&d_lens) {
    int32_t *h, *d;
    HIP_TRY(m->lens_ring.stage((size_t)N * 4, h, d));
    memcpy(h, lens, (size_t)N * 4);
    HIP_TRY(m->lens_ring.commit((size_t)N * 4, s));
    d_lens = d;
    return COCR_OK;
}

static int ensure_ctc_scratch(cocr_model *m, size_t rows) {
    if (rows <= m->ctc_lab.n && rows <= m->ctc_val.n) return COCR_OK;
    HIP_TRY(hipDeviceSynchronize());
    drop_graphs(m);
    m->amax_logits = nullptr;
    HIP_TRY(m->ctc_lab.grow(rows));
    HIP_TRY(m->ctc_val.grow(rows));
    return COCR_OK;
}

extern "C" int cocr_ctc_greedy(cocr_model *m, const float *logits, int N, int T, int ncls, const int32_t *out_lens, int32_t *labels,
                               int32_t *starts, int32_t *ends, float *conf, int32_t *counts, int max_per_line, void *stream) {
    if (!m || !logits || !out_lens || !labels || !starts || !ends || !conf || !counts) return fail(COCR_EINVAL, "null argument");
    if (N < 1 || T < 1 || ncls < 1 || max_per_line < 1) return fail(COCR_EINVAL, "empty problem");
    if (T > 8000) return fail(COCR_EUNSUPPORTED, "more than 8000 frames per line");
    HIP_TRY(hipSetDevice(m->device));
    hipStream_t s = (hipStream_t)stream;
    const int32_t *d_lens;
    int rc = upload_lens(m, out_lens, N, s, d_lens);
    if (rc) return rc;
    const bool have_argmax = logits == m->amax_logits && N * T == m->amax_rows && ncls == m->ncls;
    if (!have_argmax && (rc = ensure_ctc_scratch(m, (size_t)N * T))) return rc;
    ProfScope ps(m, s, FAM_GREEDY);
    if (!have_argmax) {
        m->amax_logits = nullptr;
        hipLaunchKernelGGL(ctc_argmax_kernel, dim3(ceil_div(N * T, 4)), dim3(256), 0, s, logits, T, ncls, N * T, d_lens, m->ctc_lab.p, m->ctc_val.p);
        LAUNCH_CHECK();
    }
    hipLaunchKernelGGL(ctc_collapse_kernel, dim3(N), dim3(64), (size_t)T * 8, s, T, d_lens, m->ctc_lab.p, m->ctc_val.p, labels, starts, ends, conf, counts,
                       max_per_line);
    LAUNCH_CHECK();
    return COCR_OK;
}

extern "C" int cocr_ctc_beam(cocr_model *m, const float *logits, int N, int T, int ncls, const int32_t *out_lens, int32_t *labels,
                             int32_t *starts, int32_t *ends, float *conf, int32_t *counts, int max_per_line, int beam, void *stream) {
    if (!m || !logits || !out_lens || !labels || !starts || !ends || !conf || !counts) return fail(COCR_EINVAL, "null argument");
    if (N < 1 || T < 1 || ncls < 2 || max_per_line < 1) return fail(COCR_EINVAL, "empty problem");
    if (beam < 1 || beam > COCR_BEAM_MAX) return fail(COCR_EINVAL, "beam must be in 1..%d", COCR_BEAM_MAX);
    if (ncls > 65535) return fail(COCR_EUNSUPPORTED, "more than 65535 classes");
    HIP_TRY(hipSetDevice(m->device));
    hipStream_t s = (hipStream_t)stream;
    const int32_t *d_lens;
    int rc = upload_lens(m, out_lens, N, s, d_lens);
    if (rc) return rc;
    const bool fast = ncls <= 256 && !m->beam_ref;
    const int K = std::min(beam + 1, ncls - 1);
    const size_t need = (size_t)N * T * ((size_t)COCR_BEAM_MAX * 4 + (fast ? (size_t)COCR_BEAM_REC : 4));
    HIP_TRY(m->beam_bp.grow(need));
    int32_t *bp = reinterpret_cast<int32_t *>(m->beam_bp.p);
    ProfScope ps(m, s, FAM_BEAM);
    if (fast) {
// ... 576 lines not shown
```

### conformer_ocr_amd/csrc/rowchain.hip.h

```cpp
#pragma once
#include <type_traits>

#include "gemm.hip.h"
#include "rowchain_args.hip.h"

#ifndef COCR_STAMP_WG
#define COCR_STAMP_WG 7
#endif
#ifndef COCR_RC_EXP
#define COCR_RC_EXP 0
#endif

__device__ __forceinline__ void swap32(float &a, float &b) { asm("s_nop 1\n\tv_permlane32_swap_b32 %0, %1" : "+v"(a), "+v"(b)); }
__device__ __forceinline__ void swap16(float &a, float &b) { asm("s_nop 1\n\tv_permlane16_swap_b32 %0, %1" : "+v"(a), "+v"(b)); }
__device__ __forceinline__ float butterfly4(float a, float b, float c, float d) {
    swap32(a, b);
    swap32(c, d);
    float ab = a + b, cd = c + d;
    swap16(ab, cd);
    return ab + cd;
}

__device__ __forceinline__ int xcd_remap_rows(int bid, int nwg) {
    const int q = nwg >> 3, r = nwg & 7, xcd = bid & 7;
    return (xcd < r ? xcd * (q + 1) : r * (q + 1) + (xcd - r) * q) + (bid >> 3);
}

#ifndef COCR_RC_PAIR
#define COCR_RC_PAIR 0
#endif
template <int D, int MT> constexpr bool rowchain_pair_form() { return COCR_RC_PAIR && D == 256 && MT == 3; }

template <int D, int MT> constexpr size_t rowchain_slack_bytes() { return rowchain_pair_form<D, MT>() ? 2048 : 4096; }
template <int D, int MT> constexpr size_t rowchain_lds_bytes() {
    return (size_t)(D / 64) * 16 * MT * 128 + 2 * 4 * (size_t)(16 * MT) * 128 + rowchain_slack_bytes<D, MT>() + 16 * (size_t)D + 12 * (size_t)(16 * MT) + 64;
}
template <int D, int MT> constexpr int rowchain_dw_pass() { return rowchain_pair_form<D, MT>() ? 128 : 256; }
template <int D, int MT, int DWK> constexpr int rowchain_taps_place() {
    if (DWK == 0 || (DWK + 1) % 8 != 0) return 0;
    constexpr size_t cw = rowchain_dw_pass<D, MT>(), rpi = 64 / (cw / 8);
    constexpr size_t hsb = 2 * 4 * (size_t)(16 * MT) * 128 + rowchain_slack_bytes<D, MT>(), win = ((16 * MT + DWK - 1 + rpi - 1) / rpi) * 1024, taps = (size_t)(DWK + 1) * cw * 4;
    if (win + taps <= hsb) return 1;
    if (rowchain_pair_form<D, MT>()) return 0;
    if (rowchain_lds_bytes<D, MT>() + taps <= 160 * 1024) return 2;
    return 0;
}

template <int D, int MT, int DWK, int K0, int K1, int K2, int K3, bool TAPS, int KD = 8, int KL = 8>
__global__ __launch_bounds__(512, (rowchain_pair_form<D, MT>() ? 4 : 2)) void rowchain_kernel(ChainArgs p) {
    typedef bf16_t T;
    static_assert(D == 256 || D == 512, "encoder_dim of the row-chain kernels");
    static_assert(MT >= 2 && MT <= 6, "16-row tiles per workgroup");
    static_assert(KD >= 1 && KD <= 8 && KL >= 1 && KL <= 8 && (D == 256 || (KD == 8 && KL == 8)), "skipped k-steps: the 256-wide engine only");
    typedef std::integral_constant<int, 8> KK8;
    typedef std::integral_constant<int, KD> KKD;
    typedef std::integral_constant<int, KL> KKL;
    typedef KKD KKQ;
    typedef KKD KKG;
    typedef KKD KKP1;
    typedef std::integral_constant<int, (K1 == ST_GLU) ? 8 : KD> KKR;
    constexpr int BMC = 16 * MT;
    constexpr int KS = D / 256;
    constexpr int NS = D / 256;
    constexpr int NJ = 2 * NS;
    constexpr int PANEL = BMC * 128;
    constexpr int IMGX = (D / 64) * PANEL;
    constexpr int IMGH = 4 * PANEL;
    constexpr int OS = 256 * 2 + 16;
    constexpr int OSD = D * 2 + 16;
    constexpr int SLICE = 16 * 512;
    constexpr int PROW = 80;
    constexpr int HSB = 2 * IMGH + (int)rowchain_slack_bytes<D, MT>();
    extern __shared__ __attribute__((aligned(16))) unsigned char smem[];
    unsigned char *xa = smem;
    unsigned char *hs = smem + IMGX;
    float *lnp = reinterpret_cast<float *>(smem + IMGX + HSB);
    long long *rowoff = reinterpret_cast<long long *>(smem + IMGX + HSB + 16 * D);
    int *tpos = reinterpret_cast<int *>(smem + IMGX + HSB + 16 * D + 8 * BMC);

    const int tid = threadIdx.x, lane = tid & 63;
    const int wave = __builtin_amdgcn_readfirstlane(tid >> 6);
    const int r16 = lane & 15, g = lane >> 4, swz = r16 & 7;
    const int rblk = p.xcd_order ? xcd_remap_rows(blockIdx.x, gridDim.x) : (int)blockIdx.x;
    const int M = p.M, m0 = rblk * BMC, mend = min(M, m0 + BMC);
    const int lrow = lane >> 3, cpos = lane & 7;
#ifdef COCR_CHAIN_STAMPS_BUILD
    int sk = 0;
#define RSTAMP() { if (p.stamps && rblk == COCR_STAMP_WG && lane == 0) p.stamps[wave * 64 + sk] = __builtin_readcyclecounter(); ++sk; }
#else
#define RSTAMP()
#endif
    RSTAMP()
    auto lds_fence_barrier = [&]() {
        asm volatile("s_waitcnt lgkmcnt(0)" ::: "memory");
        if constexpr (!(COCR_RC_EXP & 512)) __builtin_amdgcn_s_barrier();
    };

    constexpr int DWPAD = DWK ? (DWK - 1) / 2 : 0, DWROWS = BMC + 2 * DWPAD;
    constexpr int CW = rowchain_dw_pass<D, MT>();
    constexpr int WS = CW * 2;
    constexpr int LPR = CW / 8, RPI = 64 / LPR;
    constexpr int WINB = ((DWROWS + RPI - 1) / RPI) * 1024;
    static_assert(DWK == 0 || (size_t)WINB <= (size_t)HSB, "depthwise window (CW channels at a time) must fit the hidden-image area");
    static_assert((size_t)BMC * OSD <= (size_t)HSB && 2 * (size_t)BMC * OS <= (size_t)HSB, "output tiles alias the hidden-image area");
    auto dw_window = [&](int h) {
        for (int q2 = wave; q2 < WINB / 1024; q2 += 8) {
            const int j = RPI * q2 + lane / LPR, mrow = min(max(m0 - DWPAD + j, 0), M - 1);
            __builtin_amdgcn_global_load_lds((gbl_ptr_t)(p.dw_in + (size_t)mrow * D + h * CW + (lane % LPR) * 8), (lds_ptr_t)(hs + q2 * 1024), 16, 0, 0);
        }
    };
    constexpr bool FRONT0 = K0 == ST_FRONT;
    static_assert(!FRONT0 || DWK == 0, "the output linear starts a launch");
    static_assert(K1 != ST_FRONT && K2 != ST_FRONT && K3 != ST_FRONT, "FRONT is a first stage");
    auto front_dma = [&](int ks) {
        unsigned char *buf = hs + (ks & 1) * IMGH;
        const int Kf = p.st[0].K;
#pragma unroll
        for (int u = 0; u < MT; ++u) {
            const int id = wave + 8 * u, pnl = id / (BMC / 8), rg = id - pnl * (BMC / 8), row = rg * 8 + lrow;
            const T *src = p.A0 + (size_t)min(m0 + row, M - 1) * Kf + ks * 256 + pnl * 64 + ((cpos ^ (row & 7)) * 8);
            __builtin_amdgcn_global_load_lds((gbl_ptr_t)src, (lds_ptr_t)(buf + pnl * PANEL + rg * 1024), 16, 0, 0);
        }
    };
    static_assert(4 * (BMC / 8) == 8 * MT, "operand slice: MT wave-instructions per wave");
    if constexpr (FRONT0) {
        front_dma(0);
    } else if constexpr (DWK == 0) {
        for (int id = wave; id < (D / 64) * (BMC / 8); id += 8) {
            const int pnl = id / (BMC / 8), rg = id - pnl * (BMC / 8), row = rg * 8 + lrow;
            const T *src = p.A0 + (size_t)min(m0 + row, M - 1) * D + pnl * 64 + ((cpos ^ (row & 7)) * 8);
            __builtin_amdgcn_global_load_lds((gbl_ptr_t)src, (lds_ptr_t)(xa + pnl * PANEL + rg * 1024), 16, 0, 0);
        }
    } else {
        dw_window(0);
    }
    typedef float dw_f32x2 __attribute__((ext_vector_type(2)));
    dw_f32x2 dw_wt[DWK ? DWK : 1], dw_bias = {0.f, 0.f};
    constexpr int TAPLACE = rowchain_taps_place<D, MT, DWK>();
    unsigned char *tapa = TAPLACE == 1 ? hs + WINB : smem + rowchain_lds_bytes<D, MT>();
    constexpr int TPI = 256 / CW;
    auto dw_taps = [&](int h) {
        if constexpr (DWK != 0 && TAPLACE != 0) {
#pragma unroll
            for (int r2 = wave; r2 < (DWK + 1) / TPI; r2 += 8) {
                const int r = r2 * TPI + lane / (64 / TPI);
                const float *src = (r < DWK ? p.dw_w + (size_t)r * D : p.dw_b) + h * CW + (lane % (64 / TPI)) * 4;
                __builtin_amdgcn_global_load_lds((gbl_ptr_t)src, (lds_ptr_t)(tapa + r2 * 1024), 16, 0, 0);
            }
        } else if constexpr (DWK != 0) {
            const int c = h * CW + 2 * (tid % (CW / 2));
#pragma unroll
            for (int tau = 0; tau < DWK; ++tau) dw_wt[tau] = *reinterpret_cast<const dw_f32x2 *>(p.dw_w + (size_t)tau * D + c);
            dw_bias = *reinterpret_cast<const dw_f32x2 *>(p.dw_b + c);
        }
    };
    auto dw_taps_read = [&]() {
        if constexpr (DWK != 0 && TAPLACE != 0) {
            const unsigned char *tb = tapa + (tid % (CW / 2)) * 8;
#pragma unroll
            for (int tau = 0; tau < DWK; ++tau) dw_wt[tau] = *reinterpret_cast<const dw_f32x2 *>(tb + tau * (CW * 4));
            dw_bias = *reinterpret_cast<const dw_f32x2 *>(tb + DWK * (CW * 4));
        }
    };
    RSTAMP()
    dw_taps(0);
    RSTAMP()
    constexpr int RING = rowchain_pair_form<D, MT>() ? 8 : 16;
    bf16x8 ring[RING];
    auto fill = [&](const T *slice, int f) { ring[f % RING] = *reinterpret_cast<const bf16x8 *>(slice + f * 512 + lane * 8); };
    const T *cur_run = p.st[0].W + (size_t)wave * (FRONT0 ? p.st[0].K / 256 : KS) * SLICE;
    {
#pragma unroll
        for (int f = 0; f < RING; ++f) fill(cur_run, f);
    }
    __builtin_amdgcn_sched_barrier(0);
    RSTAMP()
    f32x4 xs[MT][NJ];
    const size_t xblk = ((size_t)rblk * 8 + wave) * (MT * NJ) * 256 + lane * 4;
    auto load_stream = [&]() {
        if (p.x_in_blocked) {
#pragma unroll
            for (int i = 0; i < MT; ++i)
#pragma unroll
                for (int c = 0; c < NJ; ++c) {
                    if constexpr (COCR_RC_EXP & 1) xs[i][c] = (f32x4){(float)r16, 1.f, (float)g, 0.5f};
                    else xs[i][c] = *reinterpret_cast<const f32x4 *>(p.x + xblk + (i * NJ + c) * 256);
                }
            return;
        }
#pragma unroll
        for (int i = 0; i < MT; ++i) {
            const float *xrow = p.x + (size_t)min(m0 + 16 * i + r16, mend - 1) * D + 32 * wave + 4 * g;
#pragma unroll
            for (int c = 0; c < NJ; ++c) {
                if constexpr (COCR_RC_EXP & 1) xs[i][c] = (f32x4){(float)r16, 1.f, (float)g, 0.5f};
                else xs[i][c] = *reinterpret_cast<const f32x4 *>(xrow + 256 * (c >> 1) + 16 * (c & 1));
            }
        }
    };
    constexpr int EARLY_XS = (DWK == 0 && !FRONT0) ? MT * NJ : 0;
    if constexpr (DWK == 0 && !FRONT0) load_stream();
    __builtin_amdgcn_sched_barrier(0);
    if (tid < BMC) {
        const int m = min(m0 + tid, M - 1), b = m / p.T_, t = m - b * p.T_;
        rowoff[tid] = ((long long)b * p.heads * p.Tp + t) * p.dhp;
        tpos[tid] = t;
    }
    RSTAMP()
    constexpr int RING0 = RING == 16 ? 2 * (K0 == ST_ROWLN ? KKR::value : K0 == ST_FFN ? KKP1::value : 8)
                                     : (2 * (K0 == ST_ROWLN ? KKR::value : K0 == ST_FFN ? KKP1::value : 8) < 8 ? 2 * (K0 == ST_ROWLN ? KKR::value : K0 == ST_FFN ? KKP1::value : 8) : 8);
    asm volatile("s_waitcnt vmcnt(%0)" :: "n"(RING0 + EARLY_XS) : "memory");
    lds_fence_barrier();
    RSTAMP()

    if constexpr (DWK != 0) {
        typedef float f32x2_t __attribute__((ext_vector_type(2)));
        constexpr int CPAIRS = CW / 2, NRG = 512 / CPAIRS;
        constexpr int RQ = BMC / NRG;
        constexpr int G = RQ % 8 == 0 ? 8 : (RQ % 6 == 0 ? 6 : 8);
        static_assert(BMC % NRG == 0 && RQ >= G, "rows per thread of the depthwise prologue");
        const int cp = tid % CPAIRS, rq = __builtin_amdgcn_readfirstlane(tid / CPAIRS);
        const int T_ = p.T_;
#pragma unroll 1
        for (int h = 0; h < D / CW; ++h) {
            if (h > 0) {
                dw_window(h);
                dw_taps(h);
                asm volatile("s_waitcnt vmcnt(0)" ::: "memory");
                lds_fence_barrier();
            }
            const int c = 2 * cp;
            dw_taps_read();
            const f32x2_t bias = dw_bias;
#pragma unroll 1
            for (int r0 = RQ * rq; r0 < ((COCR_RC_EXP & 2048) ? RQ * rq : RQ * (rq + 1)); r0 += G) {
                const int rb = min(r0, RQ * (rq + 1) - G);
                const int t0 = __builtin_amdgcn_readfirstlane(tpos[rb]);
                f32x2_t acc[G];
#pragma unroll
                for (int i = 0; i < G; ++i) acc[i] = bias;
                const unsigned char *wbase = hs + (size_t)rb * WS + c * 2;
                if (t0 >= DWPAD && t0 + (G - 1) + DWPAD < T_) {
#pragma unroll
                    for (int rin = 0; rin < G + DWK - 1; ++rin) {
                        const bf16x2 xv = *reinterpret_cast<const bf16x2 *>(wbase + rin * WS);
                        const f32x2_t xf = {(float)xv[0], (float)xv[1]};
#pragma unroll
                        for (int i = 0; i < G; ++i) {
                            const int tau = rin - i;
                            if (tau >= 0 && tau < DWK) { if constexpr (COCR_RC_EXP & 8) { if (tau == 0) acc[i] += xf; } else acc[i] = __builtin_elementwise_fma(dw_wt[tau], xf, acc[i]); }
                        }
                    }
                } else if (__builtin_amdgcn_readfirstlane(tpos[rb + G - 1]) == t0 + G - 1) {
#pragma unroll
                    for (int rin = 0; rin < G + DWK - 1; ++rin) {
                        const bool ok = (unsigned)(t0 + rin - DWPAD) < (unsigned)T_;
                        const bf16x2 xv = *reinterpret_cast<const bf16x2 *>(wbase + rin * WS);
                        const f32x2_t xf = {ok ? (float)xv[0] : 0.f, ok ? (float)xv[1] : 0.f};
#pragma unroll
                        for (int i = 0; i < G; ++i) {
                            const int tau = rin - i;
                            if (tau >= 0 && tau < DWK) acc[i] = __builtin_elementwise_fma(dw_wt[tau], xf, acc[i]);
                        }
                    }
                } else {
                    int ti[G];
#pragma unroll
                    for (int i = 0; i < G; ++i) ti[i] = __builtin_amdgcn_readfirstlane(tpos[rb + i]);
#pragma unroll
                    for (int rin = 0; rin < G + DWK - 1; ++rin) {
                        const bf16x2 xv = *reinterpret_cast<const bf16x2 *>(wbase + rin * WS);
                        const f32x2_t xr = {(float)xv[0], (float)xv[1]};
#pragma unroll
                        for (int i = 0; i < G; ++i) {
                            const int tau = rin - i;
                            if (tau >= 0 && tau < DWK) {
                                const bool ok = (unsigned)(ti[i] + tau - DWPAD) < (unsigned)T_;
                                const f32x2_t xf = {ok ? xr[0] : 0.f, ok ? xr[1] : 0.f};
                                acc[i] = __builtin_elementwise_fma(dw_wt[tau], xf, acc[i]);
                            }
                        }
                    }
                }
#pragma unroll
                for (int i = 0; i < G; ++i) {
                    const int row = rb + i, cc = h * CW + c;
                    const bf16x2 o = (COCR_RC_EXP & 16384) ? (bf16x2){(T)acc[i][0], (T)acc[i][1]} : (bf16x2){(T)silu_f(acc[i][0]), (T)silu_f(acc[i][1])};
                    *reinterpret_cast<bf16x2 *>(xa + (cc >> 6) * PANEL + row * 128 + ((((cc & 63) >> 3) ^ (row & 7)) << 4) + (cc & 7) * 2) = o;
                    if constexpr (TAPS) {
                        if (p.tap_dw && m0 + row < mend) *reinterpret_cast<bf16x2 *>(p.tap_dw + (size_t)(m0 + row) * D + cc) = o;
                    }
                }
            }
            lds_fence_barrier();
        }
        load_stream();
        __builtin_amdgcn_sched_barrier(0);
        RSTAMP()
    }

    auto step = [&](const unsigned char *img, auto &acc, int c0, const T *nxt, auto &&side, auto FRESH, auto KKC) {
        constexpr bool fresh = decltype(FRESH)::value;
        constexpr int KK = decltype(KKC)::value;
#pragma unroll
        for (int kk = 0; kk < KK; ++kk) {
            constexpr int HT = MT > 3 ? MT / 2 : MT;
#pragma unroll
            for (int h0 = 0; h0 < MT; h0 += HT) {
                bf16x8 a[HT];
#pragma unroll
                for (int i = 0; i < HT; ++i) {
                    if constexpr (COCR_RC_EXP & 256) { if (kk == 0) a[i] = lds_frag_swz(img + (16 * (h0 + i) + r16) * 128, 0, g, swz, T()); else asm volatile("" : "+v"(a[i])); }
                    else a[i] = lds_frag_swz(img + (kk >> 1) * PANEL + (16 * (h0 + i) + r16) * 128, kk & 1, g, swz, T());
                }
#pragma unroll
                for (int j = 0; j < 2; ++j)
#pragma unroll
                    for (int i = 0; i < HT; ++i) {
                        if constexpr (COCR_RC_EXP & 64) {
                            if (fresh && kk == 0) acc[h0 + i][c0 + j] = (f32x4){0.f, 0.f, 0.f, 0.f};
                            asm volatile("" : "+v"(acc[h0 + i][c0 + j]) : "v"(ring[2 * kk + j]), "v"(a[i]));
                        } else acc[h0 + i][c0 + j] = mma16(ring[(2 * kk + j) % RING], a[i], (fresh && kk == 0) ? (f32x4){0.f, 0.f, 0.f, 0.f} : acc[h0 + i][c0 + j]);
                    }
            }
            if constexpr (!(COCR_RC_EXP & 128)) {
                if constexpr (RING == 16) {
                    fill(nxt, 2 * kk);
                    fill(nxt, 2 * kk + 1);
                } else if (kk < 4 && kk + 4 < KK) {
                    fill(cur_run, 2 * kk + 8);
                    fill(cur_run, 2 * kk + 9);
                } else {
                    fill(nxt, 2 * (kk & 3));
                    fill(nxt, 2 * (kk & 3) + 1);
                }
            }
            side(kk);
            __builtin_amdgcn_sched_barrier(0);
        }
        if constexpr (KK < (RING == 16 ? 8 : 4) && !(COCR_RC_EXP & 128)) {
#pragma unroll
            for (int f = 2 * KK; f < RING; ++f) fill(nxt, f);
            __builtin_amdgcn_sched_barrier(0);
        }
        cur_run = nxt;
    };
    auto no_side = [](int) {};
    auto request_ln_params = [&](const ChainStage &st) {
        if (wave < 4) {
            const float *src = wave == 0 ? st.g1 : wave == 1 ? st.b1 : wave == 2 ? (st.g2 ? st.g2 : st.g1) : (st.b2 ? st.b2 : st.b1);
#pragma unroll
            for (int c = 0; c < D / 256; ++c)
                __builtin_amdgcn_global_load_lds((gbl_ptr_t)(src + c * 256 + lane * 4), (lds_ptr_t)(reinterpret_cast<unsigned char *>(lnp) + wave * D * 4 + c * 1024), 16, 0, 0);
        }
    };
    struct Bias2 { f32x4 v[2]; };
    auto load_bias = [&](const float *bias) {
        Bias2 b;
        b.v[0] = *reinterpret_cast<const f32x4 *>(bias + 32 * wave + 4 * g);
        b.v[1] = *reinterpret_cast<const f32x4 *>(bias + 32 * wave + 16 + 4 * g);
        return b;
    };
    auto add_bias_to_stream = [&](const float *bias, float alpha) {
#pragma unroll
        for (int ns = 0; ns < NS; ++ns) {
            const Bias2 b = load_bias(bias + 256 * ns);
#pragma unroll
            for (int j = 0; j < 2; ++j)
#pragma unroll
                for (int i = 0; i < MT; ++i) xs[i][2 * ns + j] += b.v[j] * alpha;
        }
    };
    auto store_stream = [&](float *dst) {
        if constexpr (COCR_RC_EXP & 2) { asm volatile("" :: "v"(xs[0][0][0])); return; }
        if (dst == p.x && p.x_out_blocked) {
#pragma unroll
            for (int i = 0; i < MT; ++i)
#pragma unroll
                for (int c = 0; c < NJ; ++c) *reinterpret_cast<f32x4 *>(dst + xblk + (i * NJ + c) * 256) = xs[i][c];
            return;
        }
#pragma unroll
        for (int i = 0; i < MT; ++i) {
            if (m0 + 16 * i + r16 < mend) {
                float *xrow = dst + (size_t)(m0 + 16 * i + r16) * D + 32 * wave + 4 * g;
#pragma unroll
                for (int c = 0; c < NJ; ++c) *reinterpret_cast<f32x4 *>(xrow + 256 * (c >> 1) + 16 * (c & 1)) = xs[i][c];
            }
        }
    };
    auto row_stats = [&](unsigned char *pbuf, bool wait_params, float (&mean)[MT], float (&rstd)[MT]) {
        if constexpr (COCR_RC_EXP & 32) { for (int i = 0; i < MT; ++i) { mean[i] = 0.f; rstd[i] = 1.f; } lds_fence_barrier(); return; }
        float s[MT], ss[MT];
#pragma unroll
        for (int i = 0; i < MT; ++i) {
            f32x4 a = xs[i][0], b = xs[i][0] * xs[i][0];
#pragma unroll
            for (int c = 1; c < NJ; ++c) { a += xs[i][c]; b = __builtin_elementwise_fma(xs[i][c], xs[i][c], b); }
            s[i] = (a[0] + a[1]) + (a[2] + a[3]);
            ss[i] = (b[0] + b[1]) + (b[2] + b[3]);
        }
#pragma unroll
        for (int i0 = 0; i0 < MT; i0 += 4) {
            const int i1 = min(i0 + 1, MT - 1), i2 = min(i0 + 2, MT - 1), i3 = min(i0 + 3, MT - 1);
            const float ts = butterfly4(s[i0], s[i1], s[i2], s[i3]), tss = butterfly4(ss[i0], ss[i1], ss[i2], ss[i3]);
            const int tile = g == 0 ? i0 : g == 1 ? i2 : g == 2 ? i1 : i3;
            *reinterpret_cast<f32x2 *>(pbuf + (16 * tile + r16) * PROW + wave * 8) = (f32x2){ts, tss};
        }
        if (wait_params && wave < 4) {
            if constexpr (KD == 8 && KL == 8) asm volatile("s_waitcnt vmcnt(%0)" :: "n"(RING) : "memory");
            else asm volatile("s_waitcnt vmcnt(0)" ::: "memory");
        }
        lds_fence_barrier();
        const float inv_d = p.inv_d;
#pragma unroll
        for (int i = 0; i < MT; ++i) {
            const unsigned char *pr = pbuf + (16 * i + r16) * PROW;
            f32x4 v = *reinterpret_cast<const f32x4 *>(pr);
            if constexpr (!(COCR_RC_EXP & 4)) {
#pragma unroll
                for (int w2 = 1; w2 < 4; ++w2) v += *reinterpret_cast<const f32x4 *>(pr + 16 * w2);
            }
            const float S = v[0] + v[2], SS = v[1] + v[3];
            mean[i] = S * inv_d;
            const float ex2 = SS * inv_d;
            rstd[i] = __builtin_amdgcn_rsqf(fmaxf(__builtin_fmaf(-mean[i], mean[i], ex2), 0.f) + 1e-5f);
        }
    };
    auto normalise = [&](int which, const float (&mean)[MT], const float (&rstd)[MT], auto IN_PLACE) {
        constexpr bool in_place = decltype(IN_PLACE)::value;
        if constexpr (COCR_RC_EXP & 8192) return;
        const float *ga = lnp + which * 2 * D, *be = ga + D;
#pragma unroll
        for (int c = 0; c < NJ; ++c) {
            const int col = 256 * (c >> 1) + 32 * wave + 16 * (c & 1) + 4 * g;
            const f32x4 gv = *reinterpret_cast<const f32x4 *>(ga + col), bv = *reinterpret_cast<const f32x4 *>(be + col);
#pragma unroll
            for (int i = 0; i < MT; ++i) {
                const float r = rstd[i], mr = -mean[i] * r;
                const f32x4 y = __builtin_elementwise_fma(__builtin_elementwise_fma(xs[i][c], (f32x4){r, r, r, r}, (f32x4){mr, mr, mr, mr}), gv, bv);
                if constexpr (in_place) {
                    xs[i][c] = y;
                } else {
                    const int row = 16 * i + r16;
                    const bf16x4 o = {(T)y[0], (T)y[1], (T)y[2], (T)y[3]};
                    *reinterpret_cast<bf16x4 *>(xa + (col >> 6) * PANEL + row * 128 + ((((col & 63) >> 3) ^ (row & 7)) << 4) + (col & 4) * 2) = o;
                }
            }
        }
    };
    auto rowln_epilogue = [&](const ChainStage &st, unsigned char *pbuf) {
        const bool chained = st.g2 != nullptr;
        if constexpr (TAPS) { if (st.tap_pre) store_stream(st.tap_pre); }
        float mean[MT], rstd[MT];
        if (!chained) {
            if (st.store_x) store_stream(p.x);
            row_stats(pbuf, true, mean, rstd);
            normalise(0, mean, rstd, std::false_type{});
        } else {
            row_stats(pbuf, true, mean, rstd);
            normalise(0, mean, rstd, std::true_type{});
            if (st.store_x) store_stream(p.x);
            if constexpr (TAPS) { if (st.tap_post) store_stream(st.tap_post); }
            row_stats(pbuf + BMC * PROW, false, mean, rstd);
            normalise(1, mean, rstd, std::false_type{});
        }
        lds_fence_barrier();
        if (st.store_xn) {
            for (int id = tid; id < BMC * (D / 8); id += 512) {
                const int row = id / (D / 8), ch = id - row * (D / 8);
                if (m0 + row < mend)
                    copy16(p.xn + (size_t)(m0 + row) * D + ch * 8, reinterpret_cast<const T *>(xa + (ch >> 3) * PANEL + row * 128 + (((ch & 7) ^ (row & 7)) << 4)));
            }
        }
    };

    auto run_stage = [&](auto KIND, auto FIRST, const ChainStage &st, const T *after) {
        constexpr int kind = decltype(KIND)::value;
        if constexpr (kind == ST_ROWLN) {
            request_ln_params(st);
            auto slice = [&](int ns, int ks) { return st.W + ((size_t)(ns * 8 + wave) * KS + ks) * SLICE; };
            if constexpr (decltype(FIRST)::value) {
                f32x4 acc[MT][NJ];
#pragma unroll
                for (int ns = 0; ns < NS; ++ns)
#pragma unroll
                    for (int ks = 0; ks < KS; ++ks) {
                        const T *nxt = ks + 1 < KS ? slice(ns, ks + 1) : (ns + 1 < NS ? slice(ns + 1, 0) : after);
                        if (ks == 0) step(xa, acc, 2 * ns, nxt, no_side, std::true_type{}, KKR{});
                        else step(xa + ks * 4 * PANEL, acc, 2 * ns, nxt, no_side, std::false_type{}, KKR{});
                    }
                add_bias_to_stream(st.bias, 1.0f);
#pragma unroll
                for (int i = 0; i < MT; ++i)
#pragma unroll
                    for (int c = 0; c < NJ; ++c) xs[i][c] += acc[i][c];
            } else {
                add_bias_to_stream(st.bias, 1.0f);
#pragma unroll
                for (int ns = 0; ns < NS; ++ns)
#pragma unroll
                    for (int ks = 0; ks < KS; ++ks)
                        step(xa + ks * 4 * PANEL, xs, 2 * ns, ks + 1 < KS ? slice(ns, ks + 1) : (ns + 1 < NS ? slice(ns + 1, 0) : after), no_side, std::false_type{}, KKR{});
            }
            RSTAMP()
            rowln_epilogue(st, hs);
            RSTAMP()
        } else if constexpr (kind == ST_FRONT) {
            static_assert(decltype(FIRST)::value, "FRONT is a first stage");
            request_ln_params(st);
            const int nsl = st.K / 256;
            auto slice = [&](int ns, int ks) { return st.W + ((size_t)(ns * 8 + wave) * nsl + ks) * SLICE; };
#pragma unroll
            for (int i = 0; i < MT; ++i)
#pragma unroll
                for (int c = 0; c < NJ; ++c) xs[i][c] = (f32x4){0.f, 0.f, 0.f, 0.f};
            add_bias_to_stream(st.bias, 1.0f);
#pragma unroll 1
            for (int ks = 0; ks < nsl; ++ks) {
                if (ks + 1 < nsl) front_dma(ks + 1);
                const unsigned char *img = hs + (ks & 1) * IMGH;
#pragma unroll
                for (int ns = 0; ns < NS; ++ns)
                    step(img, xs, 2 * ns, ns + 1 < NS ? slice(ns + 1, ks) : (ks + 1 < nsl ? slice(0, ks + 1) : after), no_side, std::false_type{}, KK8{});
                if (ks + 1 < nsl) {
                    asm volatile("s_waitcnt vmcnt(%0)" :: "n"(RING) : "memory");
                    lds_fence_barrier();
                }
            }
            RSTAMP()
            rowln_epilogue(st, hs + (nsl & 1) * IMGH);
            RSTAMP()
        } else if constexpr (kind == ST_FFN) {
            const int FF = st.N, nchunks = FF / 256;
            auto w1 = [&](int c, int ks) { return st.W + ((size_t)(c * 8 + wave) * KS + ks) * SLICE; };
            auto w2 = [&](int c, int ns) { return st.W2 + ((size_t)(ns * 8 + wave) * (FF / 32) + c * 8) * 1024; };
            f32x4 acc1[MT][2];
            Bias2 bb;
            auto silu_tile = [&](int tIdx, unsigned char *hb, auto PIN) {
                if constexpr (COCR_RC_EXP & 4096) return;
                const int i = tIdx >> 1, j = tIdx & 1;
                if constexpr (decltype(PIN)::value) asm volatile("" : "+v"(acc1[i][j]));
                const int jj = 32 * wave + 16 * j + 4 * g;
                const int ch16 = (jj & 63) >> 3, row = 16 * i + r16;
                typedef float f32x2_t __attribute__((ext_vector_type(2)));
                const f32x4 v4 = acc1[i][j] + bb.v[j];
                unsigned packed[2];
#pragma unroll
                for (int h = 0; h < 2; ++h) {
                    const f32x2_t v = {v4[2 * h], v4[2 * h + 1]};
                    f32x2_t e = v * (f32x2_t){-1.44269504088896340736f, -1.44269504088896340736f};
                    if constexpr (!(COCR_RC_EXP & 16)) e = (f32x2_t){__builtin_amdgcn_exp2f(e[0]), __builtin_amdgcn_exp2f(e[1])} + (f32x2_t){1.0f, 1.0f};
                    const f32x2_t o = (COCR_RC_EXP & 16) ? v * e : v * (f32x2_t){__builtin_amdgcn_rcpf(e[0]), __builtin_amdgcn_rcpf(e[1])};
                    packed[h] = __builtin_bit_cast(unsigned, __builtin_convertvector(o, bf16x2));
                }
                typedef unsigned u32x2_t __attribute__((ext_vector_type(2)));
                *reinterpret_cast<u32x2_t *>(hb + (jj >> 6) * PANEL + row * 128 + ((ch16 ^ (row & 7)) << 4) + ((jj & 7) >> 2) * 8) = (u32x2_t){packed[0], packed[1]};
            };
            auto p1 = [&](int c, const T *then) {
                if (wave >= 4) __builtin_amdgcn_s_setprio(1);
#pragma unroll
                for (int ks = 0; ks < KS; ++ks) {
                    if (ks == 0) step(xa, acc1, 0, KS > 1 ? w1(c, 1) : then, no_side, std::true_type{}, KKP1{});
                    else step(xa + ks * 4 * PANEL, acc1, 0, ks + 1 < KS ? w1(c, ks + 1) : then, no_side, std::false_type{}, KKP1{});
                }
                if (wave >= 4) __builtin_amdgcn_s_setprio(0);
            };
            request_ln_params(st);
            bb = load_bias(st.bias);
            p1(0, nchunks > 1 ? w1(1, 0) : w2(0, 0));
            RSTAMP()
#pragma unroll
            for (int t2 = 0; t2 < 2 * MT; ++t2) silu_tile(t2, hs, std::false_type{});
            add_bias_to_stream(st.bias2, st.alpha);
            RSTAMP()
            lds_fence_barrier();
            RSTAMP()
            for (int c = 1; c < nchunks; ++c) {
                bb = load_bias(st.bias + c * 256);
                p1(c, w2(c - 1, 0));
                RSTAMP()
                unsigned char *hb = hs + (c & 1) * IMGH;
#pragma unroll
                for (int ns = 0; ns < NS; ++ns)
                    step(hs + ((c - 1) & 1) * IMGH, xs, 2 * ns, ns + 1 < NS ? w2(c - 1, ns + 1) : (c + 1 < nchunks ? w1(c + 1, 0) : w2(c, 0)),
                         [&](int kk) {
#pragma unroll
                             for (int t2 = 0; t2 < 2 * MT; ++t2) if ((t2 * 8 * NS) / (2 * MT) == ns * 8 + kk) silu_tile(t2, hb, std::true_type{});
                         }, std::false_type{}, KK8{});
                RSTAMP()
                lds_fence_barrier();
                RSTAMP()
            }
#pragma unroll
            for (int ns = 0; ns < NS; ++ns)
                step(hs + ((nchunks - 1) & 1) * IMGH, xs, 2 * ns, ns + 1 < NS ? w2(nchunks - 1, ns + 1) : after, no_side, std::false_type{}, KKL{});
            RSTAMP()
            rowln_epilogue(st, hs + (nchunks & 1) * IMGH);
            RSTAMP()
        } else if constexpr (kind == ST_GLU) {
            EpiGLU<T> e{st.out, D, st.bias, 2 * D};
            auto slice = [&](int s2, int ks) { return st.W + ((size_t)(s2 * 8 + wave) * KS + ks) * SLICE; };
            constexpr int NSTEP = 2 * D / 256;
#pragma unroll 1
            for (int s2 = 0; s2 < NSTEP; ++s2) {
                const Bias2 bb = load_bias(st.bias + s2 * 256);
                f32x4 acc[MT][2];
#pragma unroll
                for (int ks = 0; ks < KS; ++ks) {
                    const T *nxt = ks + 1 < KS ? slice(s2, ks + 1) : (s2 + 1 < NSTEP ? slice(s2 + 1, 0) : after);
                    if (ks == 0) step(xa, acc, 0, nxt, no_side, std::true_type{}, KKG{});
                    else step(xa + ks * 4 * PANEL, acc, 0, nxt, no_side, std::false_type{}, KKG{});
                }
#pragma unroll
                for (int i = 0; i < MT; ++i) {
                    const int row = 16 * i + r16;
                    bf16x4 o;
#pragma unroll
                    for (int q = 0; q < 4; ++q) o[q] = (T)((acc[i][0][q] + bb.v[0][q]) * sigmoid_f(acc[i][1][q] + bb.v[1][q]));
                    *reinterpret_cast<bf16x4 *>(hs + row * OSD + (s2 * 128 + 16 * wave + 4 * g) * 2) = o;
                }
            }
            lds_fence_barrier();
            for (int id = tid; id < BMC * (D / 8); id += 512) {
                const int row = id / (D / 8), ch = id - row * (D / 8);
                if (m0 + row < mend) e.store(m0 + row, ch * 8, reinterpret_cast<const T *>(hs + row * OSD + ch * 16), 8);
            }
        } else if constexpr (kind == ST_QKV) {
            auto slice = [&](int s3, int ks) { return st.W + ((size_t)(s3 * 8 + wave) * KS + ks) * SLICE; };
            constexpr int NSTEP = 3 * D / 256;
#pragma unroll
            for (int s3 = 0; s3 < NSTEP; ++s3) {
                const Bias2 bb = load_bias(st.bias + s3 * 256);
                f32x4 acc[MT][2];
#pragma unroll
                for (int ks = 0; ks < KS; ++ks) {
                    const T *nxt = ks + 1 < KS ? slice(s3, ks + 1) : (s3 + 1 < NSTEP ? slice(s3 + 1, 0) : after);
                    if (ks == 0) step(xa, acc, 0, nxt, no_side, std::true_type{}, KKQ{});
                    else step(xa + ks * 4 * PANEL, acc, 0, nxt, no_side, std::false_type{}, KKQ{});
                }
                unsigned char *tile = hs + (s3 & 1) * (BMC * OS);
                if constexpr (COCR_RC_EXP & 1024) { asm volatile("" :: "v"(acc[0][0]), "v"(acc[MT - 1][1])); continue; }
#pragma unroll
                for (int j = 0; j < 2; ++j)
#pragma unroll
                    for (int i = 0; i < MT; ++i) {
                        const int row = 16 * i + r16;
                        bf16x4 o;
#pragma unroll
                        for (int q = 0; q < 4; ++q) o[q] = (T)(acc[i][j][q] + bb.v[j][q]);
                        *reinterpret_cast<bf16x4 *>(tile + row * OS + (32 * wave + 16 * j + 4 * g) * 2) = o;
                    }
                RSTAMP()
                lds_fence_barrier();
                {
                    const int which = s3 / NS;
                    T *base = which == 0 ? st.q : (which == 1 ? st.k : st.v);
                    const int ch = tid & 31, hd = (s3 - which * NS) * 256 + ch * 8, hh = hd / p.dh, d = hd - hh * p.dh;
                    base += (size_t)hh * p.Tp * p.dhp + d;
#pragma unroll
                    for (int i = 0; i < MT; ++i) {
                        const int row = (tid >> 5) + 16 * i;
                        if (m0 + row < mend) copy16(base + rowoff[row], reinterpret_cast<const T *>(tile + row * OS + ch * 16));
                    }
                }
            }
        }
    };
    auto first_slice = [&](int i) -> const T * { return p.st[i].W + (size_t)wave * ((i == 0 && FRONT0) ? p.st[0].K / 256 : KS) * SLICE; };
    run_stage(std::integral_constant<int, K0>{}, std::true_type{}, p.st[0], K1 >= 0 ? first_slice(1) : first_slice(0));
    run_stage(std::integral_constant<int, K1>{}, std::false_type{}, p.st[1], K2 >= 0 ? first_slice(2) : first_slice(0));
    run_stage(std::integral_constant<int, K2>{}, std::false_type{}, p.st[2], K3 >= 0 ? first_slice(3) : first_slice(0));
    run_stage(std::integral_constant<int, K3>{}, std::false_type{}, p.st[3], first_slice(0));
    RSTAMP()
#undef RSTAMP
}

template <int D, int MT, int DWK, int K0, int K1, int K2, int K3, bool TAPS, int KD = 8, int KL = 8>
static inline hipError_t launch_rowchain_mt(hipStream_t s, const ChainArgs &a) {
    constexpr size_t lds = rowchain_lds_bytes<D, MT>() + (rowchain_taps_place<D, MT, DWK>() == 2 ? (size_t)(DWK + 1) * 1024 : 0);
    static_assert(lds <= 160 * 1024, "LDS of one workgroup");
    auto kern = rowchain_kernel<D, MT, DWK, K0, K1, K2, K3, TAPS, KD, KL>;
    hipError_t e = raise_lds_limit((const void *)kern, lds);
    if (e != hipSuccess) return e;
    hipLaunchKernelGGL(kern, dim3(ceil_div(a.M, 16 * MT)), dim3(512), lds, s, a);
    return hipGetLastError();
}

template <int D, int DWK, int K0, int K1, int K2, int K3, bool HAS_TAPS>
static inline hipError_t launch_rowchain_cfg(hipStream_t s, const ChainArgs &a, bool taps, int rows_hint) {
    const int mt = rowchain_pick_mt<D>(a.M, rows_hint);
    if (taps && !HAS_TAPS) return hipErrorInvalidValue;
    const bool narrow = D == 256 && a.kd == 5 && a.kl == 2 && !taps;
#define COCR_RC(MTV)                                                                                            \
    if (mt == MTV) {                                                                                            \
        if constexpr (HAS_TAPS) { if (taps) return launch_rowchain_mt<D, MTV, DWK, K0, K1, K2, K3, true>(s, a); } \
        if constexpr (D == 256) { if (narrow) return launch_rowchain_mt<D, MTV, DWK, K0, K1, K2, K3, false, 5, 2>(s, a); } \
        return launch_rowchain_mt<D, MTV, DWK, K0, K1, K2, K3, false>(s, a);                                     \
    }
    if constexpr (D == 256) { COCR_RC(6) COCR_RC(4) COCR_RC(3) } else { COCR_RC(4) }
    COCR_RC(2)
#undef COCR_RC
    return hipErrorInvalidValue;
}

template <int D>
static inline hipError_t launch_rowchain(hipStream_t s, const ChainArgs &a, bool taps, int rows_hint) {
    const int k0 = a.st[0].kind, k1 = a.nstages > 1 ? a.st[1].kind : -1, k2 = a.nstages > 2 ? a.st[2].kind : -1, k3 = a.nstages > 3 ? a.st[3].kind : -1;
    if (a.dw_in) {
        if (k0 == ST_ROWLN && k1 == ST_FFN && k2 == ST_FFN && k3 == ST_QKV) return launch_rowchain_cfg<D, 31, ST_ROWLN, ST_FFN, ST_FFN, ST_QKV, true>(s, a, taps, rows_hint);
        if (k0 == ST_ROWLN && k1 == ST_FFN && k2 == -1) return launch_rowchain_cfg<D, 31, ST_ROWLN, ST_FFN, -1, -1, true>(s, a, taps, rows_hint);
        return hipErrorInvalidValue;
    }
    if (k0 == ST_FRONT && k1 == ST_FFN && k2 == ST_QKV && k3 == -1) return launch_rowchain_cfg<D, 0, ST_FRONT, ST_FFN, ST_QKV, -1, true>(s, a, taps, rows_hint);
    if (k0 == ST_FFN && k1 == ST_QKV && k2 == -1) return launch_rowchain_cfg<D, 0, ST_FFN, ST_QKV, -1, -1, true>(s, a, taps, rows_hint);
    if (k0 == ST_FFN && k1 == -1) return launch_rowchain_cfg<D, 0, ST_FFN, -1, -1, -1, false>(s, a, false, rows_hint);
    if (k0 == ST_ROWLN && k1 == ST_GLU && k2 == -1) return launch_rowchain_cfg<D, 0, ST_ROWLN, ST_GLU, -1, -1, true>(s, a, taps, rows_hint);
    if (k0 == ST_ROWLN && k1 == ST_FFN && k2 == ST_FFN && k3 == ST_QKV) return launch_rowchain_cfg<D, 0, ST_ROWLN, ST_FFN, ST_FFN, ST_QKV, true>(s, a, taps, rows_hint);
    if (k0 == ST_ROWLN && k1 == ST_FFN && k2 == -1) return launch_rowchain_cfg<D, 0, ST_ROWLN, ST_FFN, -1, -1, true>(s, a, taps, rows_hint);
    return hipErrorInvalidValue;
}
```

### conformer_ocr_amd/csrc/rowchain_args.hip.h

```cpp
#pragma once
#include <hip/hip_runtime.h>

#include <algorithm>

#include "common.hip.h"

enum { ST_ROWLN = 0, ST_FFN = 1, ST_GLU = 2, ST_QKV = 3, ST_FRONT = 4 };

struct ChainStage {
    int kind;
    const bf16_t *W;
    const bf16_t *W2;
    const float *bias;
    const float *bias2;
    int N;
    int K;
    float alpha;
    const float *g1, *b1, *g2, *b2;
    int store_x, store_xn;
    bf16_t *out;
    bf16_t *q, *k, *v;
    float *tap_pre, *tap_post;
};

struct ChainArgs {
    const bf16_t *A0;
    float *x;
    int x_in_blocked, x_out_blocked;
    bf16_t *xn;
    int M, nstages;
    int kd, kl;
    int xcd_order;
    const bf16_t *dw_in;
    const float *dw_w, *dw_b;
    bf16_t *tap_dw;
    int dh, dhp, heads, T_, Tp;
    float inv_d;
    unsigned long long *stamps;
    ChainStage st[4];
};

static inline bool rowchain_supported(int D, int FF, int dh) { return (D == 256 || D == 512) && FF % 256 == 0 && FF >= 256 && FF <= 2048 && dh % 8 == 0 && D % dh == 0; }

template <int D> static inline int rowchain_pick_mt(int M, int rows_hint) {
    constexpr int MAXMT = D == 256 ? 6 : 4;
    if (rows_hint > 0) {
        const int mt = std::min(MAXMT, std::max(2, rows_hint / 16));
        return (D == 256 && mt == 5) ? 4 : (D == 512 && mt == 3) ? 4 : mt;
    }
    if (M >= 16 * MAXMT * 50) return MAXMT;
    return 2;
}

hipError_t launch_rowchain_256(hipStream_t s, const ChainArgs &a, bool taps, int rows_hint);
hipError_t launch_rowchain_512(hipStream_t s, const ChainArgs &a, bool taps, int rows_hint);
```

Measured before the change: 36010 lines/s.

## Fuse attention out-projection and GLU head into the depthwise row-chain kernel

Adds a head stage to the 256-wide row-chain kernel. It computes the attention output projection, residual add and LayerNorm, then the pointwise GLU, for the tile rows plus one halo tile on each side. The GLU output goes straight into the LDS depthwise window, so the separate FAM_CH_A launch and the glu round-trip through global memory are gone. The residual stream now ping-pongs between two x buffers so the halo rows can be read while the new rows are written. The cost is recomputing the halo tiles, plus more LDS and registers per workgroup, which may reduce occupancy.

```diff
diff --git a/conformer_ocr_amd/csrc/cocr_api.hip b/conformer_ocr_amd/csrc/cocr_api.hip
--- a/conformer_ocr_amd/csrc/cocr_api.hip
+++ b/conformer_ocr_amd/csrc/cocr_api.hip
@@ -162,7 +162,7 @@
     int capN = 0, capW = 0;
     std::vector<void *> ws_allocs;
     void *z_a = nullptr, *z_b = nullptr;
-    float *x = nullptr;
+    float *x = nullptr, *x2 = nullptr;
     void *g_lines = nullptr;
     float *g_logits = nullptr;
     void *xn = nullptr, *hid = nullptr, *q = nullptr, *k = nullptr, *vt = nullptr, *ctx = nullptr, *glu = nullptr, *dwo = nullptr;
@@ -201,6 +201,7 @@
     bool no_front96 = false;
     bool no_front32 = false;
     bool no_dw_fuse = false;
+    bool no_a_fuse = false;
     int chain_rows = 0;
     bool no_front_chain = false;
     bool ffn_probe = false;
@@ -252,6 +253,7 @@
     {"COCR_CHAIN_XCD", &cocr_model::chain_xcd, nullptr},
     {"COCR_NO_KSKIP", &cocr_model::no_kskip, nullptr},
     {"COCR_NO_DW_FUSE", &cocr_model::no_dw_fuse, nullptr},
+    {"COCR_NO_A_FUSE", &cocr_model::no_a_fuse, nullptr},
     {"COCR_NO_FRONT96", &cocr_model::no_front96, nullptr},
     {"COCR_NO_FRONT32", &cocr_model::no_front32, nullptr},
     {"COCR_BEAM_REF", &cocr_model::beam_ref, nullptr},
@@ -787,6 +789,7 @@
     if ((rc = ws_alloc(m, &m->z_a, zbytes))) return rc;
     if ((rc = ws_alloc(m, &m->z_b, zbytes))) return rc;
     if ((rc = ws_alloc(m, (void **)&m->x, (M + 128) * m->D * 4))) return rc;
+    if ((rc = ws_alloc(m, (void **)&m->x2, (M + 128) * m->D * 4))) return rc;
     if ((rc = ws_alloc(m, &m->xn, M * m->D * es))) return rc;
     if ((rc = ws_alloc(m, &m->hid, M * m->ff * es))) return rc;
     m->qkv_bytes = (size_t)N * m->heads * Tp * m->dhp * es;
@@ -945,6 +948,7 @@
     bool chain;
     bool ffn_fused;
     bool dw_fused;
+    bool a_fused;
     bool taps;
     bool argmax;
     int chain_rows;
@@ -1005,6 +1009,7 @@
     f.dw_fused = m->ksz == 31 && (!m->no_dw_fuse || f.taps);
     f.argmax = m->ncls <= 128 && D % (128 / es) == 0;
     f.chain_rows = f.chain ? chain_rows_for(m, M) : 0;
+    f.a_fused = f.chain && f.dw_fused && !m->no_a_fuse && rowchain_head_supported(D, m->ksz, f.chain_rows);
     return f;
 }
 
@@ -1233,17 +1238,17 @@
     const size_t MD = (size_t)M * D;
     const bool taps = c.f.taps;
     int rc;
-    float *tp[4] = {nullptr, nullptr, nullptr, nullptr};
+    float *tp[5] = {nullptr, nullptr, nullptr, nullptr, nullptr};
     bf16_t *tap_dw = nullptr;
     if (taps) {
-        HIP_TRY(m->tapbuf.grow(MD * 4 + MD / 2));
-        for (int i = 0; i < 4; ++i) tp[i] = m->tapbuf.p + (size_t)i * MD;
-        tap_dw = reinterpret_cast<bf16_t *>(m->tapbuf.p + 4 * MD);
+        HIP_TRY(m->tapbuf.grow(MD * 5 + MD / 2));
+        for (int i = 0; i < 5; ++i) tp[i] = m->tapbuf.p + (size_t)i * MD;
+        tap_dw = reinterpret_cast<bf16_t *>(m->tapbuf.p + 5 * MD);
     }
     auto CW = [&](size_t off) { return (const bf16_t *)(m->packed + off); };
     auto launch = [&](const ChainArgs &a, int fam) -> int {
         ProfScope ps(m, c.s, fam);
-        GEMM_TRY(D == 256 ? launch_rowchain_256(c.s, a, taps, c.f.chain_rows) : launch_rowchain_512(c.s, a, taps, c.f.chain_rows));
+        GEMM_TRY(a.nhead ? launch_rowchain_256_head(c.s, a, taps, c.f.chain_rows) : D == 256 ? launch_rowchain_256(c.s, a, taps, c.f.chain_rows) : launch_rowchain_512(c.s, a, taps, c.f.chain_rows));
         return COCR_OK;
     };
     auto base = [&](const T *A0, int nstages) {
@@ -1286,17 +1291,23 @@
         const LayerW &w = P.layers[l];
         const bool last = l + 1 == m->L;
         if ((rc = attention(c, l, (m->stamps && l == 5) ? m->stamps + 192 : nullptr))) return rc;
-        {
+        ChainStage ha = st_rowln(w.wo, w.bo, 1.0f, w.c_ln_g, w.c_ln_b);
+        ChainStage hg{}; hg.kind = ST_GLU; hg.W = CW(w.wpw1); hg.bias = c.F32(w.bpw1); hg.N = 2 * D; hg.out = (bf16_t *)c.glu;
+        ha.tap_pre = tp[4];
+        if (!c.f.a_fused) {
             ChainArgs a = base(c.ctx, 2);
-            a.st[0] = st_rowln(w.wo, w.bo, 1.0f, w.c_ln_g, w.c_ln_b); a.st[0].store_x = 1;
-            ChainStage g{}; g.kind = ST_GLU; g.W = CW(w.wpw1); g.bias = c.F32(w.bpw1); g.N = 2 * D; g.out = (bf16_t *)c.glu;
-            a.st[1] = g;
-            a.st[0].tap_pre = tp[0];
+            a.st[0] = ha; a.st[0].store_x = 1; a.st[0].tap_pre = tp[0];
+            a.st[1] = hg;
             if ((rc = c.tap(l, "ctx", c.ctx, MD)) || (rc = launch(a, FAM_CH_A)) || (rc = c.tap_x(l, "mhsa", tp[0])) || (rc = c.tap(l, "glu", c.glu, MD))) return rc;
-        }
+        } else if ((rc = c.tap(l, "ctx", c.ctx, MD))) return rc;
         if (!c.f.dw_fused && (rc = dwconv(c, w))) return rc;
         ChainArgs a = base(c.dwo, 2);
         if (c.f.dw_fused) { a.dw_in = (const bf16_t *)c.glu; a.dw_w = c.F32(w.dww); a.dw_b = c.F32(w.dwb); a.tap_dw = tap_dw; }
+        if (c.f.a_fused) {
+            a.A0 = (const bf16_t *)c.ctx; a.dw_in = nullptr; a.nhead = 2; a.st[4] = ha; a.st[5] = hg;
+            a.xh = (l & 1) ? m->x2 : c.x; a.x = (l & 1) ? c.x : m->x2;
+            if (!taps) a.st[5].out = nullptr;
+        }
         a.st[0] = st_rowln(w.wpw2, w.bpw2, 1.0f, w.ffn[1].ln_g, w.ffn[1].ln_b);
         a.st[0].tap_pre = tp[0];
         if (!last) {
@@ -1313,6 +1324,7 @@
             a.st[1].tap_pre = tp[1];
             if ((rc = launch(a, FAM_CH_LAST))) return rc;
         }
+        if (c.f.a_fused && ((rc = c.tap_x(l, "mhsa", tp[4])) || (rc = c.tap(l, "glu", c.glu, MD)))) return rc;
         if ((rc = c.tap(l, "dw", c.f.dw_fused ? (const T *)tap_dw : (const T *)c.dwo, MD)) || (rc = c.tap_x(l, "conv", tp[0])) || (rc = c.tap_x(l, "ffn2", tp[1])))
             return rc;
         if (!last && ((rc = c.tap_x(l, "out", tp[2])) || (rc = c.tap_x(l + 1, "ffn1", tp[3])) || (rc = c.tap_qkv(l + 1)))) return rc;
diff --git a/conformer_ocr_amd/csrc/rowchain.hip.h b/conformer_ocr_amd/csrc/rowchain.hip.h
--- a/conformer_ocr_amd/csrc/rowchain.hip.h
+++ b/conformer_ocr_amd/csrc/rowchain.hip.h
@@ -32,8 +32,13 @@
 template <int D, int MT> constexpr bool rowchain_pair_form() { return COCR_RC_PAIR && D == 256 && MT == 3; }
 
 template <int D, int MT> constexpr size_t rowchain_slack_bytes() { return rowchain_pair_form<D, MT>() ? 2048 : 4096; }
-template <int D, int MT> constexpr size_t rowchain_lds_bytes() {
-    return (size_t)(D / 64) * 16 * MT * 128 + 2 * 4 * (size_t)(16 * MT) * 128 + rowchain_slack_bytes<D, MT>() + 16 * (size_t)D + 12 * (size_t)(16 * MT) + 64;
+template <int D, int MT, bool HEAD = false> constexpr size_t rowchain_area_bytes() {
+    constexpr size_t imgx = (size_t)(D / 64) * 16 * MT * 128, area = imgx + 2 * 4 * (size_t)(16 * MT) * 128 + rowchain_slack_bytes<D, MT>();
+    constexpr size_t harea = (size_t)(D / 64) * 16 * (MT + 2) * 128 + (size_t)16 * (MT + 2) * 2 * D;
+    return HEAD && harea > area ? harea : area;
+}
+template <int D, int MT, bool HEAD = false> constexpr size_t rowchain_lds_bytes() {
+    return rowchain_area_bytes<D, MT, HEAD>() + 16 * (size_t)D + 12 * (size_t)(16 * MT) + 64;
 }
 template <int D, int MT> constexpr int rowchain_dw_pass() { return rowchain_pair_form<D, MT>() ? 128 : 256; }
 template <int D, int MT, int DWK> constexpr int rowchain_taps_place() {
@@ -46,9 +51,12 @@
     return 0;
 }
 
-template <int D, int MT, int DWK, int K0, int K1, int K2, int K3, bool TAPS, int KD = 8, int KL = 8>
+template <int D, int MT, int DWK, int K0, int K1, int K2, int K3, bool TAPS, int KD = 8, int KL = 8, int H0 = -1, int H1 = -1>
 __global__ __launch_bounds__(512, (rowchain_pair_form<D, MT>() ? 4 : 2)) void rowchain_kernel(ChainArgs p) {
     typedef bf16_t T;
+    constexpr bool HEAD = H0 >= 0;
+    constexpr int ME = MT + 2;
+    static_assert(!HEAD || (H0 == ST_ROWLN && H1 == ST_GLU && K0 == ST_ROWLN && DWK == 31 && D == 256 && ME <= 6 && !rowchain_pair_form<D, MT>()), "head: out-proj -> GLU in front of the 31-tap prologue, 256 wide, at most 6 row tiles");
     static_assert(D == 256 || D == 512, "encoder_dim of the row-chain kernels");
     static_assert(MT >= 2 && MT <= 6, "16-row tiles per workgroup");
     static_assert(KD >= 1 && KD <= 8 && KL >= 1 && KL <= 8 && (D == 256 || (KD == 8 && KL == 8)), "skipped k-steps: the 256-wide engine only");
@@ -71,12 +79,14 @@
     constexpr int SLICE = 16 * 512;
     constexpr int PROW = 80;
     constexpr int HSB = 2 * IMGH + (int)rowchain_slack_bytes<D, MT>();
+    constexpr int AREA = (int)rowchain_area_bytes<D, MT, HEAD>();
+    constexpr int PANELE = 16 * ME * 128, IMGE = (D / 64) * PANELE;
     extern __shared__ __attribute__((aligned(16))) unsigned char smem[];
     unsigned char *xa = smem;
     unsigned char *hs = smem + IMGX;
-    float *lnp = reinterpret_cast<float *>(smem + IMGX + HSB);
-    long long *rowoff = reinterpret_cast<long long *>(smem + IMGX + HSB + 16 * D);
-    int *tpos = reinterpret_cast<int *>(smem + IMGX + HSB + 16 * D + 8 * BMC);
+    float *lnp = reinterpret_cast<float *>(smem + AREA);
+    long long *rowoff = reinterpret_cast<long long *>(smem + AREA + 16 * D);
+    int *tpos = reinterpret_cast<int *>(smem + AREA + 16 * D + 8 * BMC);
 
     const int tid = threadIdx.x, lane = tid & 63;
     const int wave = __builtin_amdgcn_readfirstlane(tid >> 6);
@@ -103,6 +113,17 @@
     constexpr int WINB = ((DWROWS + RPI - 1) / RPI) * 1024;
     static_assert(DWK == 0 || (size_t)WINB <= (size_t)HSB, "depthwise window (CW channels at a time) must fit the hidden-image area");
     static_assert((size_t)BMC * OSD <= (size_t)HSB && 2 * (size_t)BMC * OS <= (size_t)HSB, "output tiles alias the hidden-image area");
+    unsigned char *winx = smem + IMGE;
+    static_assert(!HEAD || (IMGE >= IMGX && IMGE + 16 * ME * WS <= AREA && CW == D && DWPAD == 15), "head: window behind both operand images");
+    const unsigned char *win = HEAD ? winx + (16 - DWPAD) * WS : hs;
+    auto head_dma = [&]() {
+#pragma unroll
+        for (int u = 0; u < (D / 64) * ME / 4; ++u) {
+            const int id = wave + 8 * u, pnl = id / (2 * ME), rg = id - pnl * (2 * ME), row = rg * 8 + lrow;
+            const T *src = p.A0 + (size_t)min(max(m0 - 16 + row, 0), M - 1) * D + pnl * 64 + ((cpos ^ (row & 7)) * 8);
+            __builtin_amdgcn_global_load_lds((gbl_ptr_t)src, (lds_ptr_t)(xa + pnl * PANELE + rg * 1024), 16, 0, 0);
+        }
+    };
     auto dw_window = [&](int h) {
         for (int q2 = wave; q2 < WINB / 1024; q2 += 8) {
             const int j = RPI * q2 + lane / LPR, mrow = min(max(m0 - DWPAD + j, 0), M - 1);
@@ -131,13 +152,16 @@
             const T *src = p.A0 + (size_t)min(m0 + row, M - 1) * D + pnl * 64 + ((cpos ^ (row & 7)) * 8);
             __builtin_amdgcn_global_load_lds((gbl_ptr_t)src, (lds_ptr_t)(xa + pnl * PANEL + rg * 1024), 16, 0, 0);
         }
+    } else if constexpr (HEAD) {
+        head_dma();
     } else {
         dw_window(0);
     }
     typedef float dw_f32x2 __attribute__((ext_vector_type(2)));
     dw_f32x2 dw_wt[DWK ? DWK : 1], dw_bias = {0.f, 0.f};
     constexpr int TAPLACE = rowchain_taps_place<D, MT, DWK>();
-    unsigned char *tapa = TAPLACE == 1 ? hs + WINB : smem + rowchain_lds_bytes<D, MT>();
+    static_assert(!HEAD || TAPLACE == 2, "head: the taps in their own area (the window is the head's to write)");
+    unsigned char *tapa = TAPLACE == 1 ? hs + WINB : smem + rowchain_lds_bytes<D, MT, HEAD>();
     constexpr int TPI = 256 / CW;
     auto dw_taps = [&](int h) {
         if constexpr (DWK != 0 && TAPLACE != 0) {
@@ -168,7 +192,7 @@
     constexpr int RING = rowchain_pair_form<D, MT>() ? 8 : 16;
     bf16x8 ring[RING];
     auto fill = [&](const T *slice, int f) { ring[f % RING] = *reinterpret_cast<const bf16x8 *>(slice + f * 512 + lane * 8); };
-    const T *cur_run = p.st[0].W + (size_t)wave * (FRONT0 ? p.st[0].K / 256 : KS) * SLICE;
+    const T *cur_run = p.st[HEAD ? 4 : 0].W + (size_t)wave * (FRONT0 ? p.st[0].K / 256 : KS) * SLICE;
     {
 #pragma unroll
         for (int f = 0; f < RING; ++f) fill(cur_run, f);
@@ -198,7 +222,18 @@
             }
         }
     };
-    constexpr int EARLY_XS = (DWK == 0 && !FRONT0) ? MT * NJ : 0;
+    f32x4 xe[HEAD ? ME : 1][NJ];
+    if constexpr (HEAD) {
+        const int nblk = gridDim.x;
+#pragma unroll
+        for (int e = 0; e < ME; ++e) {
+            const int blk = e == 0 ? max(rblk - 1, 0) : e == ME - 1 ? min(rblk + 1, nblk - 1) : rblk, tile = e == 0 ? MT - 1 : e == ME - 1 ? 0 : e - 1;
+            const float *src = p.xh + (((size_t)blk * 8 + wave) * MT + tile) * (NJ * 256) + lane * 4;
+#pragma unroll
+            for (int c = 0; c < NJ; ++c) xe[e][c] = *reinterpret_cast<const f32x4 *>(src + c * 256);
+        }
+    }
+    constexpr int EARLY_XS = HEAD ? ME * NJ : (DWK == 0 && !FRONT0) ? MT * NJ : 0;
     if constexpr (DWK == 0 && !FRONT0) load_stream();
     __builtin_amdgcn_sched_barrier(0);
     if (tid < BMC) {
@@ -207,13 +242,13 @@
         tpos[tid] = t;
     }
     RSTAMP()
-    constexpr int RING0 = RING == 16 ? 2 * (K0 == ST_ROWLN ? KKR::value : K0 == ST_FFN ? KKP1::value : 8)
+    constexpr int RING0 = HEAD ? 16 : RING == 16 ? 2 * (K0 == ST_ROWLN ? KKR::value : K0 == ST_FFN ? KKP1::value : 8)
                                      : (2 * (K0 == ST_ROWLN ? KKR::value : K0 == ST_FFN ? KKP1::value : 8) < 8 ? 2 * (K0 == ST_ROWLN ? KKR::value : K0 == ST_FFN ? KKP1::value : 8) : 8);
     asm volatile("s_waitcnt vmcnt(%0)" :: "n"(RING0 + EARLY_XS) : "memory");
     lds_fence_barrier();
     RSTAMP()
 
-    if constexpr (DWK != 0) {
+    auto dw_prologue = [&]() { if constexpr (DWK != 0) {
         typedef float f32x2_t __attribute__((ext_vector_type(2)));
         constexpr int CPAIRS = CW / 2, NRG = 512 / CPAIRS;
         constexpr int RQ = BMC / NRG;
@@ -239,7 +274,7 @@
                 f32x2_t acc[G];
 #pragma unroll
                 for (int i = 0; i < G; ++i) acc[i] = bias;
-                const unsigned char *wbase = hs + (size_t)rb * WS + c * 2;
+                const unsigned char *wbase = win + (size_t)rb * WS + c * 2;
                 if (t0 >= DWPAD && t0 + (G - 1) + DWPAD < T_) {
 #pragma unroll
                     for (int rin = 0; rin < G + DWK - 1; ++rin) {
@@ -294,24 +329,25 @@
             }
             lds_fence_barrier();
         }
-        load_stream();
+        if constexpr (!HEAD) load_stream();
         __builtin_amdgcn_sched_barrier(0);
         RSTAMP()
-    }
-
-    auto step = [&](const unsigned char *img, auto &acc, int c0, const T *nxt, auto &&side, auto FRESH, auto KKC) {
+    } };
+
+    auto step_n = [&](auto MTC, const unsigned char *img, auto &acc, int c0, const T *nxt, auto &&side, auto FRESH, auto KKC) {
+        constexpr int MTN = decltype(MTC)::value, PANELN = 16 * MTN * 128;
         constexpr bool fresh = decltype(FRESH)::value;
         constexpr int KK = decltype(KKC)::value;
 #pragma unroll
         for (int kk = 0; kk < KK; ++kk) {
-            constexpr int HT = MT > 3 ? MT / 2 : MT;
-#pragma unroll
-            for (int h0 = 0; h0 < MT; h0 += HT) {
+            constexpr int HT = (MTN > 3 && MTN % 2 == 0) ? MTN / 2 : MTN;
+#pragma unroll
+            for (int h0 = 0; h0 < MTN; h0 += HT) {
                 bf16x8 a[HT];
 #pragma unroll
                 for (int i = 0; i < HT; ++i) {
                     if constexpr (COCR_RC_EXP & 256) { if (kk == 0) a[i] = lds_frag_swz(img + (16 * (h0 + i) + r16) * 128, 0, g, swz, T()); else asm volatile("" : "+v"(a[i])); }
-                    else a[i] = lds_frag_swz(img + (kk >> 1) * PANEL + (16 * (h0 + i) + r16) * 128, kk & 1, g, swz, T());
+                    else a[i] = lds_frag_swz(img + (kk >> 1) * PANELN + (16 * (h0 + i) + r16) * 128, kk & 1, g, swz, T());
                 }
 #pragma unroll
                 for (int j = 0; j < 2; ++j)
@@ -345,6 +381,9 @@
         }
         cur_run = nxt;
     };
+    typedef std::integral_constant<int, MT> MTC0;
+    typedef std::integral_constant<int, ME> MEC;
+    auto step = [&](const unsigned char *img, auto &acc, int c0, const T *nxt, auto &&side, auto FRESH, auto KKC) { step_n(MTC0{}, img, acc, c0, nxt, side, FRESH, KKC); };
     auto no_side = [](int) {};
     auto request_ln_params = [&](const ChainStage &st) {
         if (wave < 4) {
@@ -361,16 +400,18 @@
         b.v[1] = *reinterpret_cast<const f32x4 *>(bias + 32 * wave + 16 + 4 * g);
         return b;
     };
-    auto add_bias_to_stream = [&](const float *bias, float alpha) {
+    auto add_bias_n = [&](auto MTC, auto &xs, const float *bias, float alpha) {
+        constexpr int MTN = decltype(MTC)::value;
 #pragma unroll
         for (int ns = 0; ns < NS; ++ns) {
             const Bias2 b = load_bias(bias + 256 * ns);
 #pragma unroll
             for (int j = 0; j < 2; ++j)
 #pragma unroll
-                for (int i = 0; i < MT; ++i) xs[i][2 * ns + j] += b.v[j] * alpha;
-        }
-    };
+                for (int i = 0; i < MTN; ++i) xs[i][2 * ns + j] += b.v[j] * alpha;
+        }
+    };
+    auto add_bias_to_stream = [&](const float *bias, float alpha) { add_bias_n(MTC0{}, xs, bias, alpha); };
     auto store_stream = [&](float *dst) {
         if constexpr (COCR_RC_EXP & 2) { asm volatile("" :: "v"(xs[0][0][0])); return; }
         if (dst == p.x && p.x_out_blocked) {
@@ -389,11 +430,12 @@
             }
         }
     };
-    auto row_stats = [&](unsigned char *pbuf, bool wait_params, float (&mean)[MT], float (&rstd)[MT]) {
-        if constexpr (COCR_RC_EXP & 32) { for (int i = 0; i < MT; ++i) { mean[i] = 0.f; rstd[i] = 1.f; } lds_fence_barrier(); return; }
-        float s[MT], ss[MT];
-#pragma unroll
-        for (int i = 0; i < MT; ++i) {
+    auto row_stats_n = [&](auto MTC, auto &xs, unsigned char *pbuf, bool wait_params, auto &mean, auto &rstd) {
+        constexpr int MTN = decltype(MTC)::value;
+        if constexpr (COCR_RC_EXP & 32) { for (int i = 0; i < MTN; ++i) { mean[i] = 0.f; rstd[i] = 1.f; } lds_fence_barrier(); return; }
+        float s[MTN], ss[MTN];
+#pragma unroll
+        for (int i = 0; i < MTN; ++i) {
             f32x4 a = xs[i][0], b = xs[i][0] * xs[i][0];
 #pragma unroll
             for (int c = 1; c < NJ; ++c) { a += xs[i][c]; b = __builtin_elementwise_fma(xs[i][c], xs[i][c], b); }
@@ -401,8 +443,8 @@
             ss[i] = (b[0] + b[1]) + (b[2] + b[3]);
         }
 #pragma unroll
-        for (int i0 = 0; i0 < MT; i0 += 4) {
-            const int i1 = min(i0 + 1, MT - 1), i2 = min(i0 + 2, MT - 1), i3 = min(i0 + 3, MT - 1);
+        for (int i0 = 0; i0 < MTN; i0 += 4) {
+            const int i1 = min(i0 + 1, MTN - 1), i2 = min(i0 + 2, MTN - 1), i3 = min(i0 + 3, MTN - 1);
             const float ts = butterfly4(s[i0], s[i1], s[i2], s[i3]), tss = butterfly4(ss[i0], ss[i1], ss[i2], ss[i3]);
             const int tile = g == 0 ? i0 : g == 1 ? i2 : g == 2 ? i1 : i3;
             *reinterpret_cast<f32x2 *>(pbuf + (16 * tile + r16) * PROW + wave * 8) = (f32x2){ts, tss};
@@ -414,7 +456,7 @@
         lds_fence_barrier();
         const float inv_d = p.inv_d;
 #pragma unroll
-        for (int i = 0; i < MT; ++i) {
+        for (int i = 0; i < MTN; ++i) {
             const unsigned char *pr = pbuf + (16 * i + r16) * PROW;
             f32x4 v = *reinterpret_cast<const f32x4 *>(pr);
             if constexpr (!(COCR_RC_EXP & 4)) {
@@ -427,7 +469,9 @@
             rstd[i] = __builtin_amdgcn_rsqf(fmaxf(__builtin_fmaf(-mean[i], mean[i], ex2), 0.f) + 1e-5f);
         }
     };
-    auto normalise = [&](int which, const float (&mean)[MT], const float (&rstd)[MT], auto IN_PLACE) {
+    auto row_stats = [&](unsigned char *pbuf, bool wait_params, float (&mean)[MT], float (&rstd)[MT]) { row_stats_n(MTC0{}, xs, pbuf, wait_params, mean, rstd); };
+    auto normalise_n = [&](auto MTC, auto &xs, int which, const auto &mean, const auto &rstd, auto IN_PLACE) {
+        constexpr int MTN = decltype(MTC)::value, PANELN = 16 * MTN * 128;
         constexpr bool in_place = decltype(IN_PLACE)::value;
         if constexpr (COCR_RC_EXP & 8192) return;
         const float *ga = lnp + which * 2 * D, *be = ga + D;
@@ -436,7 +480,7 @@
             const int col = 256 * (c >> 1) + 32 * wave + 16 * (c & 1) + 4 * g;
             const f32x4 gv = *reinterpret_cast<const f32x4 *>(ga + col), bv = *reinterpret_cast<const f32x4 *>(be + col);
 #pragma unroll
-            for (int i = 0; i < MT; ++i) {
+            for (int i = 0; i < MTN; ++i) {
                 const float r = rstd[i], mr = -mean[i] * r;
                 const f32x4 y = __builtin_elementwise_fma(__builtin_elementwise_fma(xs[i][c], (f32x4){r, r, r, r}, (f32x4){mr, mr, mr, mr}), gv, bv);
                 if constexpr (in_place) {
@@ -444,11 +488,12 @@
                 } else {
                     const int row = 16 * i + r16;
                     const bf16x4 o = {(T)y[0], (T)y[1], (T)y[2], (T)y[3]};
-                    *reinterpret_cast<bf16x4 *>(xa + (col >> 6) * PANEL + row * 128 + ((((col & 63) >> 3) ^ (row & 7)) << 4) + (col & 4) * 2) = o;
-                }
-            }
-        }
-    };
+                    *reinterpret_cast<bf16x4 *>(xa + (col >> 6) * PANELN + row * 128 + ((((col & 63) >> 3) ^ (row & 7)) << 4) + (col & 4) * 2) = o;
+                }
+            }
+        }
+    };
+    auto normalise = [&](int which, const float (&mean)[MT], const float (&rstd)[MT], auto IN_PLACE) { normalise_n(MTC0{}, xs, which, mean, rstd, IN_PLACE); };
     auto rowln_epilogue = [&](const ChainStage &st, unsigned char *pbuf) {
         const bool chained = st.g2 != nullptr;
         if constexpr (TAPS) { if (st.tap_pre) store_stream(st.tap_pre); }
@@ -668,6 +713,70 @@
         }
     };
     auto first_slice = [&](int i) -> const T * { return p.st[i].W + (size_t)wave * ((i == 0 && FRONT0) ? p.st[0].K / 256 : KS) * SLICE; };
+    auto run_head = [&]() { if constexpr (HEAD) {
+        const ChainStage &hr = p.st[4], &hg = p.st[5];
+        auto gslice = [&](int s2) { return hg.W + (size_t)(s2 * 8 + wave) * SLICE; };
+        request_ln_params(hr);
+        {
+            f32x4 acc[ME][NJ];
+            step_n(MEC{}, xa, acc, 0, gslice(0), no_side, std::true_type{}, KK8{});
+            add_bias_n(MEC{}, xe, hr.bias, 1.0f);
+#pragma unroll
+            for (int i = 0; i < ME; ++i)
+#pragma unroll
+                for (int c = 0; c < NJ; ++c) xe[i][c] += acc[i][c];
+        }
+        RSTAMP()
+        if constexpr (TAPS) {
+            if (hr.tap_pre) {
+#pragma unroll
+                for (int i = 0; i < MT; ++i) {
+                    if (m0 + 16 * i + r16 < mend) {
+                        float *xrow = hr.tap_pre + (size_t)(m0 + 16 * i + r16) * D + 32 * wave + 4 * g;
+#pragma unroll
+                        for (int c = 0; c < NJ; ++c) *reinterpret_cast<f32x4 *>(xrow + 256 * (c >> 1) + 16 * (c & 1)) = xe[i + 1][c];
+                    }
+                }
+            }
+        }
+        {
+            float mean[ME], rstd[ME];
+            row_stats_n(MEC{}, xe, winx, true, mean, rstd);
+            normalise_n(MEC{}, xe, 0, mean, rstd, std::false_type{});
+        }
+        lds_fence_barrier();
+#pragma unroll
+        for (int i = 0; i < MT; ++i)
+#pragma unroll
+            for (int c = 0; c < NJ; ++c) xs[i][c] = xe[i + 1][c];
+        RSTAMP()
+#pragma unroll 1
+        for (int s2 = 0; s2 < 2; ++s2) {
+            const Bias2 bb = load_bias(hg.bias + s2 * 256);
+            f32x4 acc[ME][2];
+            step_n(MEC{}, xa, acc, 0, s2 == 0 ? gslice(1) : first_slice(0), no_side, std::true_type{}, KKG{});
+#pragma unroll
+            for (int i = 0; i < ME; ++i) {
+                const int row = 16 * i + r16;
+                bf16x4 o;
+#pragma unroll
+                for (int q = 0; q < 4; ++q) o[q] = (T)((acc[i][0][q] + bb.v[0][q]) * sigmoid_f(acc[i][1][q] + bb.v[1][q]));
+                *reinterpret_cast<bf16x4 *>(winx + row * WS + (s2 * 128 + 16 * wave + 4 * g) * 2) = o;
+            }
+        }
+        lds_fence_barrier();
+        if constexpr (TAPS) {
+            if (hg.out) {
+                for (int id = tid; id < BMC * (D / 8); id += 512) {
+                    const int row = id / (D / 8), ch = id - row * (D / 8);
+                    if (m0 + row < mend) copy16(hg.out + (size_t)(m0 + row) * D + ch * 8, reinterpret_cast<const T *>(winx + (16 + row) * WS + ch * 16));
+                }
+            }
+        }
+        RSTAMP()
+    } };
+    run_head();
+    dw_prologue();
     run_stage(std::integral_constant<int, K0>{}, std::true_type{}, p.st[0], K1 >= 0 ? first_slice(1) : first_slice(0));
     run_stage(std::integral_constant<int, K1>{}, std::false_type{}, p.st[1], K2 >= 0 ? first_slice(2) : first_slice(0));
     run_stage(std::integral_constant<int, K2>{}, std::false_type{}, p.st[2], K3 >= 0 ? first_slice(3) : first_slice(0));
@@ -676,11 +785,11 @@
 #undef RSTAMP
 }
 
-template <int D, int MT, int DWK, int K0, int K1, int K2, int K3, bool TAPS, int KD = 8, int KL = 8>
+template <int D, int MT, int DWK, int K0, int K1, int K2, int K3, bool TAPS, int KD = 8, int KL = 8, int H0 = -1, int H1 = -1>
 static inline hipError_t launch_rowchain_mt(hipStream_t s, const ChainArgs &a) {
-    constexpr size_t lds = rowchain_lds_bytes<D, MT>() + (rowchain_taps_place<D, MT, DWK>() == 2 ? (size_t)(DWK + 1) * 1024 : 0);
+    constexpr size_t lds = rowchain_lds_bytes<D, MT, (H0 >= 0)>() + (rowchain_taps_place<D, MT, DWK>() == 2 ? (size_t)(DWK + 1) * 1024 : 0);
     static_assert(lds <= 160 * 1024, "LDS of one workgroup");
-    auto kern = rowchain_kernel<D, MT, DWK, K0, K1, K2, K3, TAPS, KD, KL>;
+    auto kern = rowchain_kernel<D, MT, DWK, K0, K1, K2, K3, TAPS, KD, KL, H0, H1>;
     hipError_t e = raise_lds_limit((const void *)kern, lds);
     if (e != hipSuccess) return e;
     hipLaunchKernelGGL(kern, dim3(ceil_div(a.M, 16 * MT)), dim3(512), lds, s, a);
@@ -704,9 +813,34 @@
     return hipErrorInvalidValue;
 }
 
+template <int K2, int K3>
+static inline hipError_t launch_rowchain_head_cfg(hipStream_t s, const ChainArgs &a, bool taps, int rows_hint) {
+    const int mt = rowchain_pick_mt<256>(a.M, rows_hint);
+    const bool narrow = a.kd == 5 && a.kl == 2 && !taps;
+#define COCR_RC(MTV)                                                                                                                \
+    if (mt == MTV) {                                                                                                                \
+        if (taps) return launch_rowchain_mt<256, MTV, 31, ST_ROWLN, ST_FFN, K2, K3, true, 8, 8, ST_ROWLN, ST_GLU>(s, a);              \
+        if (narrow) return launch_rowchain_mt<256, MTV, 31, ST_ROWLN, ST_FFN, K2, K3, false, 5, 2, ST_ROWLN, ST_GLU>(s, a);           \
+        return launch_rowchain_mt<256, MTV, 31, ST_ROWLN, ST_FFN, K2, K3, false, 8, 8, ST_ROWLN, ST_GLU>(s, a);                       \
+    }
+    COCR_RC(4) COCR_RC(3) COCR_RC(2)
+#undef COCR_RC
+    return hipErrorInvalidValue;
+}
+template <int D>
+static inline hipError_t launch_rowchain_head(hipStream_t s, const ChainArgs &a, bool taps, int rows_hint) {
+    static_assert(D == 256, "the head: encoder_dim 256");
+    const int k0 = a.st[0].kind, k1 = a.nstages > 1 ? a.st[1].kind : -1, k2 = a.nstages > 2 ? a.st[2].kind : -1, k3 = a.nstages > 3 ? a.st[3].kind : -1;
+    if (a.nhead != 2 || a.st[4].kind != ST_ROWLN || a.st[5].kind != ST_GLU || !a.dw_w || !a.A0 || !a.xh || a.xh == a.x || !a.x_in_blocked) return hipErrorInvalidValue;
+    if (k0 == ST_ROWLN && k1 == ST_FFN && k2 == ST_FFN && k3 == ST_QKV) return launch_rowchain_head_cfg<ST_FFN, ST_QKV>(s, a, taps, rows_hint);
+    if (k0 == ST_ROWLN && k1 == ST_FFN && k2 == -1) return launch_rowchain_head_cfg<-1, -1>(s, a, taps, rows_hint);
+    return hipErrorInvalidValue;
+}
+
 template <int D>
 static inline hipError_t launch_rowchain(hipStream_t s, const ChainArgs &a, bool taps, int rows_hint) {
     const int k0 = a.st[0].kind, k1 = a.nstages > 1 ? a.st[1].kind : -1, k2 = a.nstages > 2 ? a.st[2].kind : -1, k3 = a.nstages > 3 ? a.st[3].kind : -1;
+    if (a.nhead) return hipErrorInvalidValue;
     if (a.dw_in) {
         if (k0 == ST_ROWLN && k1 == ST_FFN && k2 == ST_FFN && k3 == ST_QKV) return launch_rowchain_cfg<D, 31, ST_ROWLN, ST_FFN, ST_FFN, ST_QKV, true>(s, a, taps, rows_hint);
         if (k0 == ST_ROWLN && k1 == ST_FFN && k2 == -1) return launch_rowchain_cfg<D, 31, ST_ROWLN, ST_FFN, -1, -1, true>(s, a, taps, rows_hint);
diff --git a/conformer_ocr_amd/csrc/rowchain_args.hip.h b/conformer_ocr_amd/csrc/rowchain_args.hip.h
--- a/conformer_ocr_amd/csrc/rowchain_args.hip.h
+++ b/conformer_ocr_amd/csrc/rowchain_args.hip.h
@@ -26,9 +26,11 @@
 struct ChainArgs {
     const bf16_t *A0;
     float *x;
+    const float *xh;
     int x_in_blocked, x_out_blocked;
     bf16_t *xn;
     int M, nstages;
+    int nhead;
     int kd, kl;
     int xcd_order;
     const bf16_t *dw_in;
@@ -37,7 +39,7 @@
     int dh, dhp, heads, T_, Tp;
     float inv_d;
     unsigned long long *stamps;
-    ChainStage st[4];
+    ChainStage st[6];
 };
 
 static inline bool rowchain_supported(int D, int FF, int dh) { return (D == 256 || D == 512) && FF % 256 == 0 && FF >= 256 && FF <= 2048 && dh % 8 == 0 && D % dh == 0; }
@@ -54,3 +56,5 @@
 
 hipError_t launch_rowchain_256(hipStream_t s, const ChainArgs &a, bool taps, int rows_hint);
 hipError_t launch_rowchain_512(hipStream_t s, const ChainArgs &a, bool taps, int rows_hint);
+hipError_t launch_rowchain_256_head(hipStream_t s, const ChainArgs &a, bool taps, int rows_hint);
+static inline bool rowchain_head_supported(int D, int conv_kernel, int rows) { return D == 256 && conv_kernel == 31 && rows >= 32 && rows <= 64; }
diff --git a/conformer_ocr_amd/csrc/rowchain_d256_head.hip b/conformer_ocr_amd/csrc/rowchain_d256_head.hip
--- /dev/null
+++ b/conformer_ocr_amd/csrc/rowchain_d256_head.hip
@@ -0,0 +1,3 @@
+#include "rowchain.hip.h"
+
+hipError_t launch_rowchain_256_head(hipStream_t s, const ChainArgs &a, bool taps, int rows_hint) { return launch_rowchain_head<256>(s, a, taps, rows_hint); }
```

After: 37260 lines/s (median of 6 runs). +3.4%, better.
